# frankyeh/UNet-Studio

Hardware: AMD Instinct MI355X
Metric: voxels/sec 3D U-Net train step @128^3 bf16 (higher is better)
Workload: dtype bf16

## Files before the change

### unet-studio_amd/csrc/device_util.h

```cpp
#pragma once
#include <hip/hip_bf16.h>
#include <hip/hip_runtime.h>
#include <cstdint>

#include "kernels.h"

namespace unet {

typedef __hip_bfloat16 bf16;

template <typename T> __device__ __forceinline__ float ld(const T* p, int64_t i);
template <> __device__ __forceinline__ float ld<float>(const float* p, int64_t i) { return p[i]; }
template <> __device__ __forceinline__ float ld<bf16>(const bf16* p, int64_t i) { return __bfloat162float(p[i]); }
template <typename T> __device__ __forceinline__ void st(T* p, int64_t i, float v);
template <> __device__ __forceinline__ void st<float>(float* p, int64_t i, float v) { p[i] = v; }
template <> __device__ __forceinline__ void st<bf16>(bf16* p, int64_t i, float v) { p[i] = __float2bfloat16(v); }

__device__ __forceinline__ float act_f(float v, int act) {
    switch (act) {
        case 1: return v > 0.f ? v : 0.f;
        case 2: return v > 0.f ? v : 0.01f * v;
        case 3: return v > 0.f ? v : expm1f(v);
        default: return v;
    }
// ... 42 lines not shown
}

constexpr int BRICK_X = 16, BRICK_Y = 4, BRICK_Z = 4;

__device__ __forceinline__ bool brick_walk(int W, int H, int D, int gx, int gy, int& x, int& y, int& z) {
    const unsigned nb = gridDim.x, per = (nb + 7) / 8;
    const unsigned b = (blockIdx.x & 7) * per + (blockIdx.x >> 3);
    if (b >= nb) { x = y = z = 0; return false; }
    const unsigned bx = b % gx, r = b / gx, by = r % gy, bz = r / gy;
    x = bx * BRICK_X + (threadIdx.x & (BRICK_X - 1));
    y = by * BRICK_Y + ((threadIdx.x / BRICK_X) & (BRICK_Y - 1));
    z = bz * BRICK_Z + threadIdx.x / (BRICK_X * BRICK_Y);
    return x < W && y < H && z < D;
}

struct Tri {
    unsigned o[8];
    float tx, ty, tz;
    bool ok;
};

__device__ __forceinline__ Tri locate(float x, float y, float z, int W, int H, int D) {
#pragma clang fp contract(off)
    Tri t;
    t.ok = (x >= 0.f) && (y >= 0.f) && (z >= 0.f) && (x <= (float)(W - 1)) && (y <= (float)(H - 1)) && (z <= (float)(D - 1));
    if (!t.ok) return t;
    float fx = floorf(x), fy = floorf(y), fz = floorf(z);
    t.tx = x - fx; t.ty = y - fy; t.tz = z - fz;
    const int x0 = (int)fx, y0 = (int)fy, z0 = (int)fz;
    const int x1 = min(x0 + 1, W - 1), y1 = min(y0 + 1, H - 1), z1 = min(z0 + 1, D - 1);
    const unsigned r00 = (unsigned)(z0 * H + y0) * (unsigned)W, r10 = (unsigned)(z0 * H + y1) * (unsigned)W,
                   r01 = (unsigned)(z1 * H + y0) * (unsigned)W, r11 = (unsigned)(z1 * H + y1) * (unsigned)W;
    t.o[0] = r00 + x0; t.o[1] = r00 + x1; t.o[2] = r10 + x0; t.o[3] = r10 + x1;
    t.o[4] = r01 + x0; t.o[5] = r01 + x1; t.o[6] = r11 + x0; t.o[7] = r11 + x1;
    return t;
}

__device__ __forceinline__ float lerp1(float t, float a, float b) {
#pragma clang fp contract(off)
    return a + t * (b - a);
}

__device__ __forceinline__ float trilinear(const Tri& t, const float* __restrict__ vol) {
    float c00 = lerp1(t.tx, vol[t.o[0]], vol[t.o[1]]);
    float c10 = lerp1(t.tx, vol[t.o[2]], vol[t.o[3]]);
    float c01 = lerp1(t.tx, vol[t.o[4]], vol[t.o[5]]);
    float c11 = lerp1(t.tx, vol[t.o[6]], vol[t.o[7]]);
    return lerp1(t.tz, lerp1(t.ty, c00, c10), lerp1(t.ty, c01, c11));
}

__device__ __forceinline__ float majority(const Tri& t, const float* __restrict__ vol) {
#pragma clang fp contract(off)
    float v[8], w[8];
    float wx[2] = {1.0f - t.tx, t.tx}, wy[2] = {1.0f - t.ty, t.ty}, wz[2] = {1.0f - t.tz, t.tz};
#pragma unroll
    for (int i = 0; i < 8; ++i) {
        v[i] = vol[t.o[i]];
        w[i] = wx[i & 1] * wy[(i >> 1) & 1] * wz[i >> 2];
    }
    float best = v[0], best_score = -1.f;
#pragma unroll
    for (int j = 0; j < 8; ++j) {
        float s = 0.f;
#pragma unroll
        for (int i = 0; i < 8; ++i) s += (v[i] == v[j]) ? w[i] : 0.f;
        if (s > best_score) { best_score = s; best = v[j]; }
    }
    return best;
}

__device__ __forceinline__ void pp_acc(float x, float& m, float& s, float& sf, float fgc) {
    if (x > m) {
        const float e = expf(m - x);
        s = s * e + 1.f;
        sf = sf * e + fgc;
        m = x;
    } else if (x != -INFINITY) {
        const float e = expf(x - m);
        s += e;
        sf += fgc * e;
    }
}

static inline unsigned cdiv64(int64_t a, int64_t b) { return (unsigned)((a + b - 1) / b); }

}
```

### unet-studio_amd/csrc/engine.cpp

```cpp
#include <hip/hip_runtime.h>

#include <algorithm>
#include <atomic>
#include <cmath>
#include <cstdio>
#include <cstring>
#include <functional>
#include <stdexcept>
#include <string>
#include <mutex>
#include <random>
#include <unordered_map>
#include <vector>

#include "../../include/unet_hip.h"
#include "conv_select.h"
#include "graph.hpp"
#include "kernels.h"

using namespace unet;

namespace {

thread_local std::string g_err;
int fail(const std::string& m) { g_err = m; return 1; }

#define HIP_OK(expr)                                                                              \
    do {                                                                                          \
        hipError_t e_ = (expr);                                                                   \
        if (e_ != hipSuccess) throw std::runtime_error(std::string(#expr) + ": " + hipGetErrorString(e_)); \
    } while (0)

struct DeviceGuard {
    int prev = -1;
    explicit DeviceGuard(int dev) {
        HIP_OK(hipGetDevice(&prev));
        if (prev != dev) HIP_OK(hipSetDevice(dev));
        else prev = -1;
    }
    ~DeviceGuard() { if (prev >= 0) (void)hipSetDevice(prev); }
};

size_t align_up(size_t v, size_t a = 256) { return (v + a - 1) / a * a; }

struct EnvSwitches {
    bool no_side_stream = getenv("UNET_NO_SIDE_STREAM"), no_first_wgrad_fuse = getenv("UNET_NO_FIRST_WGRAD_FUSE"), op_polite = getenv("UNET_OP_POLITE");
};
const EnvSwitches& env() { static const EnvSwitches e; return e; }

struct ProfRec { int op, cat; hipEvent_t e0, e1; };
struct ProfSink { std::vector<ProfRec> recs; };
thread_local ProfSink* g_prof = nullptr;
struct ProfScope {
    ProfRec r{};
    hipStream_t s = nullptr;
    bool on = false;
    ProfScope(int op, int cat, hipStream_t st) {
        if (!g_prof) return;
        on = true; s = st; r.op = op; r.cat = cat;
        if (hipEventCreate(&r.e0) != hipSuccess || hipEventCreate(&r.e1) != hipSuccess) { on = false; return; }
        (void)hipEventRecord(r.e0, s);
    }
    ~ProfScope() {
        if (!on) return;
        (void)hipEventRecord(r.e1, s);
        g_prof->recs.push_back(r);
    }
};

}

struct unet_plan {
    Graph g;
    int dtype = 0, device = 0, impl = 0;
    size_t elsize = 4;
    std::vector<size_t> t_off, g_off;
    std::vector<size_t> a_off;
    std::vector<size_t> n_stat, n_coef;
    std::vector<size_t> w_fwd, w_dgrad;
    std::vector<size_t> wm_fwd, wm_dgrad;
    std::vector<int> n_consumers;
    std::vector<int> first_consumer;
    mutable std::mutex bn_mu;
    mutable std::unordered_map<const void*, std::pair<int, int>> bn_pending;
    mutable std::unordered_map<const void*, std::vector<int>> bn_done;
    std::vector<ConvChoice> conv;
    size_t wgrad_off = 0;
    std::vector<size_t> wz_off;
    std::vector<int> wz_job_of_op;
    std::vector<WgradReduceJob> wz_jobs;
    WgradReduceJob* wz_jobs_dev = nullptr;
    size_t partial_off = 0, partial_bytes = 0;
    size_t ws_bytes = 0;
    size_t loss_bytes = 0;
    std::vector<int64_t> p_off;
    std::vector<PackJob> pack_jobs;
    int64_t pack_blocks = 0;
    PackJob* jobs_dev = nullptr;
    SgdSeg* segs_dev = nullptr;
    int nseg = 0;
    int64_t n_param_elems = 0;

    hipStream_t side = nullptr;
    hipEvent_t ev_fork = nullptr, ev_join = nullptr, ev_pack = nullptr, ev_packd = nullptr;
    int pack_split_op = 0;
    int64_t pack_split_blocks = 0, pack_fwd_blocks = 0;
    size_t head_off = 0;
    size_t deep_part_off = 0, deep_part_bytes = 0, deep_cnt_off = 0;
    static constexpr int deep_ncnt = 4096;
    std::vector<size_t> head_op_off;

    ~unet_plan() {
        if (segs_dev) (void)hipFree(segs_dev);
        if (wz_jobs_dev) (void)hipFree(wz_jobs_dev);
        if (jobs_dev) (void)hipFree(jobs_dev);
        if (ev_fork) (void)hipEventDestroy(ev_fork);
        if (ev_join) (void)hipEventDestroy(ev_join);
        if (ev_pack) (void)hipEventDestroy(ev_pack);
        if (ev_packd) (void)hipEventDestroy(ev_packd);
        if (side) (void)hipStreamDestroy(side);
    }

    ConvGeom op_geom_of(const Op& op) const {
        const Tensor& a = g.tensors[op.src[0]];
        const Tensor& o = g.tensors[op.dst];
        ConvGeom cg;
        cg.Cin = op.cin; cg.Cout = op.cout; cg.D = a.D; cg.H = a.H; cg.W = a.W; cg.Do = o.D; cg.Ho = o.H; cg.Wo = o.W;
        cg.ks = op.ks; cg.stride = op.stride;
        return cg;
    }
    void src_chans(const Op& op, SrcDesc* sd) const {
        for (int k = 0; k < op.nsrc; ++k) sd[k].C = g.tensors[op.src[k]].C;
    }
    std::vector<int> side_polite;
    std::vector<char> wgrad_on_main;
    void choose_polite() {
        side_polite.assign(g.ops.size(), 0);
        wgrad_on_main.assign(g.ops.size(), 0);
        bool first = true, any_deep = false;
        for (size_t i = 0; i < g.ops.size(); ++i) {
            const Op& op = g.ops[i];
            if (op.kind != OP_CONV && op.kind != OP_CONVT) continue;
            if (g.tensors[op.dst].voxels() <= (int64_t)32 * 32 * 32) { any_deep = true; break; }
            if (!first && op.kind == OP_CONV && op.stride == 2) wgrad_on_main[i] = 1;
            first = false;
        }
        if (!any_deep) return;
        for (size_t i = 0; i < g.ops.size(); ++i) {
            const Op& op = g.ops[i];
            if (op.kind == OP_CONV || op.kind == OP_CONVT) side_polite[i] = wgrad_on_main[i] ? 0 : 1;
        }
    }

    bool head_only(size_t t) const {
        if (dtype != UNET_DTYPE_BF16 || g.tensors[t].norm < 0 || g.tensors[t].C % 16) return false;
        int readers = 0;
        for (size_t i = 0; i < g.ops.size(); ++i) {
            const Op& op = g.ops[i];
            if (op.kind == OP_NORM) continue;
            for (int k = 0; k < op.nsrc; ++k) {
                if (op.src[k] != (int)t) continue;
                if (conv[i].fwd != Fwd::head) return false;
                ++readers;
            }
        }
        return readers > 0;
    }
    void layout() {
        choose_polite();
        conv.assign(g.ops.size(), ConvChoice());
        for (size_t i = 0; i < g.ops.size(); ++i) {
            const Op& op = g.ops[i];
            if (op.kind != OP_CONV && op.kind != OP_CONVT) continue;
            SrcDesc sd[2];
            src_chans(op, sd);
            conv[i] = choose_conv(dtype, impl, op_geom_of(op), sd, op.nsrc, op.out_level >= 0, op.kind == OP_CONVT);
        }
        size_t off = 0;
        auto take = [&](size_t bytes) { size_t o = off; off = align_up(off + bytes); return o; };
        t_off.assign(g.tensors.size(), SIZE_MAX);
        g_off.assign(g.tensors.size(), SIZE_MAX);
        n_consumers.assign(g.tensors.size(), 0);
        first_consumer.assign(g.tensors.size(), -1);
        for (size_t oi = 0; oi < g.ops.size(); ++oi) {
            const Op& op = g.ops[oi];
            for (int k = 0; k < op.nsrc && op.kind != OP_NORM; ++k)
                if (op.src[k] >= 0) { ++n_consumers[op.src[k]]; if (first_consumer[op.src[k]] < 0) first_consumer[op.src[k]] = (int)oi; }
        }
        a_off.assign(g.tensors.size(), SIZE_MAX);
        for (size_t i = 0; i < g.tensors.size(); ++i) {
            t_off[i] = take((size_t)g.tensors[i].numel() * elsize);
            if (g.tensors[i].needs_grad) g_off[i] = take((size_t)g.tensors[i].numel() * elsize);
            if (impl == UNET_IMPL_AUTO && (g.tensors[i].norm >= 0 || g.tensors[i].act != ACT_NONE) && !head_only(i))
                a_off[i] = take((size_t)g.tensors[i].numel() * elsize);
        }
        n_stat.resize(g.norms.size()); n_coef.resize(g.norms.size());
        size_t pmax = 0;
        for (size_t i = 0; i < g.norms.size(); ++i) {
            n_stat[i] = take(4 * (size_t)g.norms[i].C * 4);
            n_coef[i] = take(3 * (size_t)g.norms[i].C * 4);
            size_t pb = (size_t)stats_blocks(g.tensors[g.norms[i].tensor].voxels()) * g.norms[i].C * 2 * (dtype == UNET_DTYPE_F32 ? 8 : 4);
            if (pb > pmax) pmax = pb;
        }
        w_fwd.assign(g.ops.size(), SIZE_MAX); w_dgrad.assign(g.ops.size(), SIZE_MAX);
        wm_fwd.assign(g.ops.size(), SIZE_MAX); wm_dgrad.assign(g.ops.size(), SIZE_MAX);
        auto grow = [](size_t& m, size_t b) { if (b > m) m = b; };
        for (size_t i = 0; i < g.ops.size(); ++i) {
            const Op& op = g.ops[i];
            if (op.kind != OP_CONV && op.kind != OP_CONVT) continue;
            const ConvChoice& c = conv[i];
            const ConvGeom cg = op_geom_of(op);
            int k3 = op.kind == OP_CONV ? op.ks * op.ks * op.ks : 8;
            w_fwd[i] = take((size_t)k3 * op.cin * round_up(op.cout, 8) * 4);
            w_dgrad[i] = take((size_t)k3 * op.cout * round_up(op.cin, 8) * 4);
            if (op.kind == OP_CONVT) {
                if (c.mfma_fwd()) { wm_fwd[i] = take(mfma_convt_w_bytes(cg)); wm_dgrad[i] = take(mfma_convt_dgrad_w_bytes(cg)); }
                continue;
            }
            const bool stats = g.tensors[op.dst].norm >= 0;
            SrcDesc sd[2];
            src_chans(op, sd);
            if (c.mfma_fwd()) {
                wm_fwd[i] = take(mfma_conv_w_bytes(cg));
                if (stats) grow(pmax, (size_t)mfma_conv_blocks(cg) * op.cout * 2 * 4);
            }
            if (c.fwd == Fwd::first_f32_mfma && stats) grow(pmax, (size_t)conv_first_f32_mfma_blocks(cg) * op.cout * 2 * 8);
            if (c.fwd == Fwd::f32_mfma && stats) grow(pmax, (size_t)conv_f32_mfma_stat_rows(cg, sd) * op.cout * 2 * 8);
            if (c.dgrad == Dgrad::mfma) {
                wm_dgrad[i] = take(mfma_conv_dgrad_w_bytes(cg));
                if (op.stride == 2) grow(pmax, (size_t)s2_conv_dgrad_rows_max() * op.cin * 2 * 4);
            }
        }
        partial_bytes = pmax ? pmax : 256;
        partial_off = take(partial_bytes);
        size_t wmax = 0, hmax = 0;
        for (size_t i = 0; i < g.ops.size(); ++i) {
            const Op& op = g.ops[i];
            if (op.kind != OP_CONV && op.kind != OP_CONVT) continue;
            const ConvChoice& c = conv[i];
            const ConvGeom cg = op_geom_of(op);
            grow(wmax, wgrad_direct_scratch_bytes(cg, op.kind == OP_CONVT));
            if (op.kind == OP_CONVT) {
                if (c.wgrad == Wgrad::mfma) {
                    grow(wmax, mfma_convt_wgrad_scratch_bytes(cg));
                    grow(wmax, bias_grad_scratch_bytes(cg.Cout, (int64_t)cg.Do * cg.Ho * cg.Wo));
                }
                continue;
            }
            if (c.wgrad == Wgrad::mfma) grow(wmax, mfma_wgrad_scratch_bytes(cg, side_polite[i]));
            if (c.wgrad == Wgrad::f32_mfma) grow(wmax, wgrad_f32_mfma_scratch_bytes(cg));
            if (wgrad_small_supported(cg, op.nsrc)) grow(wmax, wgrad_small_scratch_bytes(cg));
            if (cg.Cin == 1 && (cg.Cout == 16 || cg.Cout == 32)) grow(wmax, conv_first_wgrad_mfma_scratch_bytes(cg));
            if (head_supported(cg, op.nsrc)) grow(hmax, head_bwd_scratch_bytes(cg));
        }
        wgrad_off = take(wmax ? wmax : 256);
        head_off = take(hmax ? hmax : 256);
        if (dtype == UNET_DTYPE_BF16 && impl == UNET_IMPL_AUTO) {
            deep_part_bytes = (size_t)8 << 20;
            deep_part_off = take(deep_part_bytes);
            deep_cnt_off = take((size_t)deep_ncnt * 4);
        }
        head_op_off.assign(g.ops.size(), SIZE_MAX);
        for (size_t i = 0; i < g.ops.size(); ++i)
            if (conv[i].fwd == Fwd::head) head_op_off[i] = take(head_bwd_scratch_bytes(op_geom_of(g.ops[i])));
        wz_off.assign(g.ops.size(), SIZE_MAX);
        for (size_t i = 0; i < g.ops.size(); ++i) {
            const Op& op = g.ops[i];
            const Wgrad w = conv[i].wgrad;
            if (op.out_level >= 0 || (w != Wgrad::first_mfma && w != Wgrad::mfma)) continue;
            const ConvGeom cg = op_geom_of(op);
            if (w == Wgrad::first_mfma) wz_off[i] = take(conv_first_wgrad_mfma_scratch_bytes(cg));
            else if (op.kind == OP_CONV) { if (!mfma_conv_wgrad_direct(cg)) wz_off[i] = take(mfma_wgrad_scratch_bytes(cg, side_polite[i])); }
            else if (!mfma_convt_wgrad_direct(cg)) wz_off[i] = take(mfma_convt_wgrad_scratch_bytes(cg));
        }
        ws_bytes = off;
        p_off.assign(g.params.size() + 1, 0);
        for (size_t i = 0; i < g.params.size(); ++i) {
            int64_t n = 1;
            for (auto d : g.params[i].shape) n *= d;
            p_off[i + 1] = p_off[i] + n;
        }
        wz_jobs.clear();
        wz_job_of_op.assign(g.ops.size(), -1);
        int wz_blk = 0;
        for (size_t i = 0; i < g.ops.size(); ++i) {
            if (wz_off[i] == SIZE_MAX) continue;
            const Op& op = g.ops[i];
            ConvGeom cg = op_geom_of(op);
            WgradReduceJob j;
            j.op = (int)i;
            j.slab_off = (long long)(wz_off[i] / 4);
            j.dw_off = p_off[op.weight];
            j.Cb = op.cout;
            if (op.kind == OP_CONVT) {
                j.nsplit = mfma_convt_wgrad_splits(cg);
                j.n = (long long)8 * op.cin * op.cout;
                j.bias_off = op.bias >= 0 ? j.slab_off + (long long)j.nsplit * j.n : -1;
                j.db_off = op.bias >= 0 ? p_off[op.bias] : -1;
            } else {
                j.nsplit = conv[i].wgrad == Wgrad::first_mfma ? conv_first_wgrad_splits(cg) : mfma_conv_wgrad_splits(cg, side_polite[i]);
                j.n = (long long)27 * op.cin * op.cout;
                j.bias_off = op.bias >= 0 ? j.slab_off + (long long)j.nsplit * j.n : -1;
                j.db_off = op.bias >= 0 ? p_off[op.bias] : -1;
            }
            wz_blk += wgrad_reduce_job_blocks(j, wz_blk);
            wz_job_of_op[i] = (int)wz_jobs.size();
            wz_jobs.push_back(j);
        }
        pack_jobs.clear();
        pack_blocks = 0;
        pack_split_op = -1; pack_split_blocks = 0; pack_fwd_blocks = 0;
        for (int which = 0; which < 2; ++which) {
            for (size_t i = 0; i < g.ops.size(); ++i) {
                const Op& op = g.ops[i];
                if (!conv[i].mfma_fwd()) continue;
                if (which == 0 && pack_split_op < 0 && g.tensors[op.dst].voxels() <= (int64_t)16 * 16 * 16) { pack_split_op = (int)i; pack_split_blocks = pack_blocks; }
                PackJob jb[2];
                int n = op.kind == OP_CONV ? mfma_conv_pack_jobs(op_geom_of(op), conv[i].dgrad == Dgrad::mfma, jb) : mfma_convt_pack_jobs(op_geom_of(op), jb);
                if (which >= n) continue;
                jb[which].src_off = p_off[op.weight];
                jb[which].dst_off = (int64_t)(which == 0 ? wm_fwd[i] : wm_dgrad[i]);
                jb[which].blk0 = pack_blocks;
                pack_blocks += jb[which].total;
                pack_jobs.push_back(jb[which]);
            }
            if (which == 0) pack_fwd_blocks = pack_blocks;
        }
    }
};

namespace {

void norm_fwd_passes(int dtype, const void* raw, int C, int64_t S, float* partial, int rows, bool dbl, bool eval, const float* gamma,
                     const float* beta, double eps, float* stat, float* rm, float* rv, int act, void* act_out, hipStream_t s) {
    if (eval) launch_norm_eval(C, gamma, beta, rm, rv, eps, stat, s);
    else {
        if (!rows) {
            launch_stats_partial(dtype, raw, C, S, partial, s);
            rows = stats_blocks(S);
            dbl = dtype == UNET_DTYPE_F32;
        }
        if (!dbl && act_out && launch_norm_finalize_apply(dtype, partial, rows, C, S, gamma, beta, eps, stat, rm, rv, 0.1, raw, act, act_out, s))
            return;
        launch_norm_finalize(partial, rows, C, S, gamma, beta, eps, stat, rm, rv, 0.1, s, dbl);
    }
    if (act_out) {
        SrcDesc d;
        d.ptr = raw; d.C = C; d.act = act; d.scale = stat + 2 * C; d.shift = stat + 3 * C;
        launch_apply_view(dtype, d, act_out, S, s);
    }
}
void norm_bwd_passes(int dtype, void* g, const void* u, int C, int64_t S, const float* stat, int act, const float* gamma, float* coef,
                     float* dgamma, float* dbeta, float* partial, int rows, bool no_apply, hipStream_t s) {
    if (rows <= 0) {
        launch_norm_bwd_partial(dtype, g, u, C, S, stat, act, partial, s);
        rows = stats_blocks(S);
    }
    if (!no_apply && launch_norm_bwd_finalize_apply(dtype, partial, rows, C, S, gamma, stat, coef, dgamma, dbeta, g, u, act, s)) return;
    launch_norm_bwd_finalize(partial, rows, C, S, gamma, stat, coef, dgamma, dbeta, s, dtype == UNET_DTYPE_F32);
    if (!no_apply) launch_norm_bwd_apply(dtype, g, u, C, S, stat, coef, act, s);
}

struct Exec {
    const unet_plan& p;
    char* ws;
    hipStream_t s;
    bool deep_on = false;
    Exec(const unet_plan& plan, void* workspace, void* stream) : p(plan), ws((char*)workspace), s((hipStream_t)stream) {}
    DeepScratch deep() const {
        DeepScratch d;
        if (deep_on && p.deep_part_bytes) { d.part = (float*)(ws + p.deep_part_off); d.part_bytes = p.deep_part_bytes; d.cnt = (int*)(ws + p.deep_cnt_off); d.ncnt = p.deep_ncnt; }
        return d;
    }
    int* deep_cnt() const { return p.deep_part_bytes ? (int*)(ws + p.deep_cnt_off) : nullptr; }

    void* tptr(int t) const { return ws + p.t_off[t]; }
    void* gptr(int t) const { return p.g_off[t] == SIZE_MAX ? nullptr : ws + p.g_off[t]; }
    float* stat(int n) const { return (float*)(ws + p.n_stat[n]); }
    float* coef(int n) const { return (float*)(ws + p.n_coef[n]); }
    float* partial() const { return (float*)(ws + p.partial_off); }

    SrcDesc raw_src(int t) const {
        const Tensor& T = p.g.tensors[t];
        SrcDesc d;
        d.ptr = tptr(t); d.C = T.C; d.act = T.act;
        if (T.norm >= 0) { d.scale = stat(T.norm) + 2 * T.C; d.shift = stat(T.norm) + 3 * T.C; }
        return d;
    }
    SrcDesc src(int t) const {
        if (p.a_off[t] == SIZE_MAX) return raw_src(t);
        SrcDesc d;
        d.ptr = ws + p.a_off[t]; d.C = p.g.tensors[t].C;
        return d;
    }
    void apply_view(int t) const {
        if (p.a_off[t] != SIZE_MAX) launch_apply_view(p.dtype, raw_src(t), ws + p.a_off[t], p.g.tensors[t].voxels(), s);
    }
    ConvGeom geom(const Op& op) const { return p.op_geom_of(op); }

    void forward(const float* const* params, float* const* buffers, const float* x, float* const* outs, int mode,
                 const std::function<void(int)>* on_head = nullptr) {
        const Graph& g = p.g;
        const bool packs_current = (mode & UNET_MODE_PACKS_CURRENT) != 0;
        mode &= 1;
        std::vector<int> fused_blocks(g.norms.size(), 0);
        std::vector<char> fused_dbl(g.norms.size(), 0);
        std::vector<char> fused_done(g.norms.size(), 0);
        bool packed = false, pack_pending = false, pack2_pending = false;
        if (p.jobs_dev && packs_current) { packed = true; deep_on = true; }
        else if (p.jobs_dev) {
            bool flat = true;
            for (size_t i = 0; i < g.params.size() && flat; ++i) flat = params[i] == params[0] + p.p_off[i];
            if (flat) {
                const int njobs = (int)p.pack_jobs.size();
                if (mode == 1 && p.side && !env().no_side_stream && !g_prof) {
                    HIP_OK(hipEventRecord(p.ev_fork, s));
                    HIP_OK(hipStreamWaitEvent(p.side, p.ev_fork, 0));
                    if (p.pack_split_op > 0 && p.pack_split_blocks > 0) {
                        launch_mfma_pack_batched(params[0], ws, p.jobs_dev, njobs, p.pack_split_blocks, p.side, 0, 0, deep_cnt(), p.deep_ncnt);
                        HIP_OK(hipEventRecord(p.ev_join, p.side));
                        launch_mfma_pack_batched(params[0], ws, p.jobs_dev, njobs, p.pack_fwd_blocks - p.pack_split_blocks, p.side, p.pack_split_blocks);
                        HIP_OK(hipEventRecord(p.ev_pack, p.side));
                        pack2_pending = true;
                        launch_mfma_pack_batched(params[0], ws, p.jobs_dev, njobs, p.pack_blocks - p.pack_fwd_blocks, p.side, p.pack_fwd_blocks);
                        HIP_OK(hipEventRecord(p.ev_packd, p.side));
                    } else {
                        launch_mfma_pack_batched(params[0], ws, p.jobs_dev, njobs, p.pack_blocks, p.side, 0, 0, deep_cnt(), p.deep_ncnt);
                        HIP_OK(hipEventRecord(p.ev_join, p.side));
                    }
                    pack_pending = true;
                } else {
                    ProfScope ps(-1, UNET_PROF_OTHER, s);
                    launch_mfma_pack_batched(params[0], ws, p.jobs_dev, njobs, mode == 1 ? p.pack_blocks : p.pack_fwd_blocks, s, 0, 0, deep_cnt(), p.deep_ncnt);
                }
                packed = true;
                deep_on = true;
            }
        }
        auto need_packs = [&](int op_index = 1 << 30) {
            if (pack_pending) { HIP_OK(hipStreamWaitEvent(s, p.ev_join, 0)); pack_pending = false; }
            if (pack2_pending && op_index >= p.pack_split_op) { HIP_OK(hipStreamWaitEvent(s, p.ev_pack, 0)); pack2_pending = false; }
        };
        for (size_t i = 0; i < g.ops.size(); ++i) {
            const Op& op = g.ops[i];
            ProfScope ps((int)i, (op.kind == OP_CONV || op.kind == OP_CONVT) ? UNET_PROF_CONV_FWD : op.kind == OP_NORM ? UNET_PROF_NORM_FWD : UNET_PROF_OTHER, s);
            switch (op.kind) {
                case OP_PACK_INPUT:
                    launch_pack_input(p.dtype, x, tptr(op.dst), g.in_c, g.tensors[op.dst].voxels(), s);
                    break;
                case OP_CONV:
                case OP_CONVT: {
                    if (op.out_level >= 0 && !(outs && outs[op.out_level])) break;
                    SrcDesc sd[2] = {src(op.src[0]), op.nsrc > 1 ? src(op.src[1]) : SrcDesc()};
                    ConvGeom cg = geom(op);
                    float* wf = (float*)(ws + p.w_fwd[i]);
                    float* wd = (float*)(ws + p.w_dgrad[i]);
                    const int k3 = op.ks * op.ks * op.ks;
                    const ConvChoice& c = p.conv[i];
                    const Tensor& T = g.tensors[op.dst];
                    const bool want_stats = T.norm >= 0 && !(g.norms[T.norm].batch && mode == 0);
                    if (op.kind == OP_CONVT) {
                        if (c.mfma_fwd()) {
                            need_packs((int)i);
                            if (!packed) launch_mfma_pack_convt_w(params[op.weight], ws + p.wm_fwd[i], mode == 1 ? ws + p.wm_dgrad[i] : nullptr, cg, s);
                            if (!(deep_on && launch_deep_convt_fwd(cg, sd, op.nsrc, ws + p.wm_fwd[i], params[op.bias], tptr(op.dst), deep(), s)))
                                launch_mfma_convt_fwd(cg, sd, op.nsrc, ws + p.wm_fwd[i], params[op.bias], tptr(op.dst), s);
                            break;
                        }
                        if (!packs_current) launch_pack_convt_w(params[op.weight], wf, wd, op.cin, op.cout, s);
                        if (c.fwd == Fwd::f32_mfma) launch_convt_f32_mfma(cg, sd, wf, params[op.bias], (float*)tptr(op.dst), s);
                        else launch_convt_fwd_direct(p.dtype, cg, sd, op.nsrc, wf, params[op.bias], tptr(op.dst), s);
                        break;
                    }
                    float* const part = want_stats ? partial() : nullptr;
                    int rows = 0;
                    switch (c.fwd) {
                        case Fwd::deep:
                        case Fwd::mfma:
                            need_packs((int)i);
                            if (!packed)
                                launch_mfma_pack_conv_w(params[op.weight], ws + p.wm_fwd[i],
                                                        (mode == 1 && c.dgrad == Dgrad::mfma) ? ws + p.wm_dgrad[i] : nullptr, cg, s);
                            if (mode == 1 && c.dgrad != Dgrad::mfma && !packs_current) launch_pack_conv_w(params[op.weight], wf, wd, op.cin, op.cout, k3, s);
                            if (c.fwd == Fwd::deep && deep_on) {
                                DeepNormFwd nf;
                                const bool fuse = T.norm >= 0 && p.a_off[op.dst] != SIZE_MAX;
                                if (fuse) {
                                    const Norm& n = g.norms[T.norm];
                                    nf = {params[n.gamma], params[n.beta], n.eps, stat(T.norm), n.batch ? buffers[n.buffer] : nullptr,
                                          n.batch ? buffers[n.buffer + 1] : nullptr, 0.1, (n.batch && mode == 0) ? 1 : 0, T.act, ws + p.a_off[op.dst]};
                                }
                                if (launch_deep_conv_fwd(cg, sd, op.nsrc, ws + p.wm_fwd[i], params[op.bias], tptr(op.dst), fuse ? &nf : nullptr, deep(), s)) {
                                    if (fuse) fused_done[T.norm] = 1;
                                    break;
                                }
                            }
                            rows = launch_mfma_conv_fwd(cg, sd, op.nsrc, ws + p.wm_fwd[i], params[op.bias], tptr(op.dst), part, s);
                            break;
                        case Fwd::head:
                            launch_head_fwd(p.dtype, cg, sd[0], params[op.weight], params[op.bias], outs[op.out_level] ? nullptr : tptr(op.dst),
                                            outs[op.out_level], s);
                            break;
                        case Fwd::first_mfma:
                            rows = launch_conv_first_mfma(cg, sd, params[op.weight], params[op.bias], tptr(op.dst), part, s);
                            if (mode == 1 && !packs_current && g.tensors[op.src[0]].needs_grad)
                                launch_pack_conv_w(params[op.weight], wf, wd, op.cin, op.cout, k3, s);
                            break;
                        case Fwd::first_f32_mfma:
                            rows = launch_conv_first_f32_mfma(cg, sd, params[op.weight], params[op.bias], (float*)tptr(op.dst), (double*)part, s);
                            if (mode == 1 && !packs_current) launch_pack_conv_w(params[op.weight], wf, wd, op.cin, op.cout, k3, s);
                            break;
                        case Fwd::f32_mfma:
                            if (!packs_current) launch_pack_conv_w(params[op.weight], wf, wd, op.cin, op.cout, k3, s);
                            rows = launch_conv_f32_mfma(cg, sd, op.nsrc, wf, params[op.bias], (float*)tptr(op.dst), s, (double*)part);
                            break;
                        case Fwd::direct:
                            if (!packs_current) launch_pack_conv_w(params[op.weight], wf, wd, op.cin, op.cout, k3, s);
                            launch_conv_fwd_direct(p.dtype, cg, sd, op.nsrc, wf, params[op.bias], tptr(op.dst),
                                                   op.out_level >= 0 ? outs[op.out_level] : nullptr, s);
                            break;
                    }
                    if (want_stats) {
                        fused_blocks[T.norm] = rows;
                        fused_dbl[T.norm] = c.fwd == Fwd::first_f32_mfma || c.fwd == Fwd::f32_mfma;
                    }
                    break;
                }
                case OP_NORM: {
                    const Norm& n = g.norms[op.norm];
                    const Tensor& T = g.tensors[n.tensor];
                    if (fused_done[op.norm]) break;
                    norm_fwd_passes(p.dtype, tptr(n.tensor), n.C, T.voxels(), partial(), fused_blocks[op.norm], fused_dbl[op.norm] != 0,
                                    n.batch && mode == 0, params[n.gamma], params[n.beta], n.eps, stat(op.norm),
                                    n.batch ? buffers[n.buffer] : nullptr, n.batch ? buffers[n.buffer + 1] : nullptr, T.act,
                                    p.a_off[n.tensor] != SIZE_MAX ? ws + p.a_off[n.tensor] : nullptr, s);
                    break;
                }
                case OP_MATERIALIZE: {
                    SrcDesc sd[2] = {src(op.src[0]), op.nsrc > 1 ? src(op.src[1]) : SrcDesc()};
                    launch_materialize(p.dtype, sd, op.nsrc, tptr(op.dst), g.tensors[op.dst].voxels(), s);
                    break;
                }
                case OP_MAXPOOL: {
                    const Tensor& a = g.tensors[op.src[0]];
                    launch_maxpool_fwd(p.dtype, src(op.src[0]), tptr(op.dst), a.D, a.H, a.W, s);
                    break;
                }
                case OP_UPSAMPLE: {
                    const Tensor& a = g.tensors[op.src[0]];
                    launch_upsample_fwd(p.dtype, src(op.src[0]), tptr(op.dst), a.D, a.H, a.W, s);
                    break;
                }
                case OP_EXPORT:
                    if (outs && outs[op.out_level])
                        launch_export(p.dtype, src(op.src[0]), outs[op.out_level], g.tensors[op.src[0]].voxels(), s);
                    break;
            }
            if (op.kind != OP_NORM && op.kind != OP_EXPORT && op.dst >= 0) {
                const Tensor& T = g.tensors[op.dst];
                if (T.norm < 0 && T.act != ACT_NONE) apply_view(op.dst);
            }
            if (on_head && op.out_level >= 0 && outs && outs[op.out_level] && (op.kind == OP_CONV || op.kind == OP_CONVT || op.kind == OP_EXPORT))
                (*on_head)(op.out_level);
        }
        need_packs();
    }

    void view_backward(int t, const float* const* params, float* const* gparams, bool no_apply = false) {
        const Tensor& T = p.g.tensors[t];
        if (T.norm >= 0) {
            const Norm& n = p.g.norms[T.norm];
            int have = 0;
            {
                std::lock_guard<std::mutex> lk(p.bn_mu);
                auto d = p.bn_done.find(ws);
                if (d != p.bn_done.end()) {
                    auto f = std::find(d->second.begin(), d->second.end(), t);
                    if (f != d->second.end()) { d->second.erase(f); return; }
                }
                auto it = p.bn_pending.find(ws);
                if (it != p.bn_pending.end()) { if (it->second.first == t) have = it->second.second; p.bn_pending.erase(it); }
            }
            norm_bwd_passes(p.dtype, gptr(t), tptr(t), T.C, T.voxels(), stat(T.norm), T.act, params[n.gamma], coef(T.norm),
                            gparams[n.gamma], gparams[n.beta], partial(), have, no_apply, s);
        } else if (T.act != ACT_NONE) {
            launch_act_bwd(p.dtype, gptr(t), tptr(t), T.act, T.numel(), s);
        }
    }

    void backward(const float* const* params, const float* const* grad_outs, float* const* gparams, float* grad_x, int op_hi = 1 << 30,
                  int op_lo = 0) {
        const Graph& g = p.g;
        if (p.side) HIP_OK(hipStreamWaitEvent(s, p.ev_packd, 0));
        {
            bool flat = p.jobs_dev != nullptr;
            for (size_t k = 0; k < g.params.size() && flat; ++k) flat = params[k] == params[0] + p.p_off[k];
            deep_on = flat;
        }
        std::vector<char> init(g.tensors.size(), 0);
        auto dst_of = [&](int t) {
            DstGrad d;
            d.C = g.tensors[t].C;
            d.ptr = g.tensors[t].needs_grad ? gptr(t) : nullptr;
            d.accumulate = init[t];
            return d;
        };
        auto mark = [&](const Op& op) {
            for (int k = 0; k < op.nsrc; ++k)
                if (g.tensors[op.src[k]].needs_grad) init[op.src[k]] = 1;
        };
        const hipStream_t sb = (p.side && !env().no_side_stream && !g_prof) ? p.side : s;
        auto fork = [&]() {
            if (sb == s) return;
            HIP_OK(hipEventRecord(p.ev_fork, s));
            HIP_OK(hipStreamWaitEvent(sb, p.ev_fork, 0));
        };
        if (op_lo < 0) op_lo = 0;
        if (op_hi >= (int)g.ops.size()) { std::lock_guard<std::mutex> lk(p.bn_mu); p.bn_pending.erase(ws); p.bn_done.erase(ws); }
// ... 720 lines not shown
        g.stride = 2; g.Do = (D - 1) / 2 + 1; g.Ho = (H - 1) / 2 + 1; g.Wo = (W - 1) / 2 + 1;
        w = std::max(mfma_wgrad_scratch_bytes(g, 0), mfma_wgrad_scratch_bytes(g, 1));
        if (w > b) b = w;
        g.Do = 2 * D; g.Ho = 2 * H; g.Wo = 2 * W;
        w = mfma_convt_wgrad_scratch_bytes(g);
        if (w > b) b = w;
    }
    *bytes = b;
    return 0;
}

static ConvGeom op_geom(int cin, int cout, int D, int H, int W, int ks, int stride, bool transposed) {
    ConvGeom g;
    g.Cin = cin; g.Cout = cout; g.D = D; g.H = H; g.W = W; g.ks = ks; g.stride = stride;
    if (transposed) { g.Do = 2 * D; g.Ho = 2 * H; g.Wo = 2 * W; }
    else {
        int pad = (ks - 1) / 2;
        g.Do = (D + 2 * pad - ks) / stride + 1; g.Ho = (H + 2 * pad - ks) / stride + 1; g.Wo = (W + 2 * pad - ks) / stride + 1;
    }
    return g;
}
static void op_pack(const float* w, int cin, int cout, int k3, bool transposed, void* scratch, float** wf, float** wd, hipStream_t s) {
    *wf = (float*)scratch; *wd = (float*)((char*)scratch + OpScratch(cin, cout).half);
    if (transposed) launch_pack_convt_w(w, *wf, *wd, cin, cout, s);
    else launch_pack_conv_w(w, *wf, *wd, cin, cout, k3, s);
}
#define OP_TRY(...) try { __VA_ARGS__; check_launch(); return 0; } catch (const std::exception& e) { return fail(e.what()); }
static DeepScratch op_deep() {
    static std::mutex mu;
    static std::unordered_map<int, DeepScratch> per_dev;
    int dev = 0;
    HIP_OK(hipGetDevice(&dev));
    std::lock_guard<std::mutex> lk(mu);
    auto it = per_dev.find(dev);
    if (it != per_dev.end()) return it->second;
    DeepScratch d;
    d.part_bytes = (size_t)8 << 20; d.ncnt = 4096;
    char* base = nullptr;
    HIP_OK(hipMalloc((void**)&base, d.part_bytes + (size_t)d.ncnt * 4));
    HIP_OK(hipMemset(base + d.part_bytes, 0, (size_t)d.ncnt * 4));
    d.part = (float*)base; d.cnt = (int*)(base + d.part_bytes);
    per_dev[dev] = d;
    return d;
}

int unet_op_conv3d_fwd(int dtype, int impl, const void* x, const float* w, const float* b, void* y, int cin, int cout, int D, int H,
                       int W, int ks, int stride, void* scratch, void* stream) {
    OP_TRY({
        hipStream_t s = (hipStream_t)stream;
        ConvGeom g = op_geom(cin, cout, D, H, W, ks, stride, false);
        float *wf, *wd;
        SrcDesc sd; sd.ptr = x; sd.C = cin;
        const ConvChoice c = choose_conv(dtype, impl, g, &sd, 1, false, false);
        if (c.mfma_fwd()) {
            void* wm = (char*)scratch + OpScratch(cin, cout).pack;
            launch_mfma_pack_conv_w(w, wm, nullptr, g, s);
            if (!launch_deep_conv_fwd(g, &sd, 1, wm, b, y, nullptr, op_deep(), s)) launch_mfma_conv_fwd(g, &sd, 1, wm, b, y, nullptr, s);
        } else if (c.fwd == Fwd::first_mfma) {
            launch_conv_first_mfma(g, &sd, w, b, y, nullptr, s);
        } else if (c.fwd == Fwd::first_f32_mfma) {
            (void)launch_conv_first_f32_mfma(g, &sd, w, b, (float*)y, nullptr, s);
        } else {
            op_pack(w, cin, cout, ks * ks * ks, false, scratch, &wf, &wd, s);
            if (c.fwd == Fwd::f32_mfma) (void)launch_conv_f32_mfma(g, &sd, 1, wf, b, (float*)y, s);
            else launch_conv_fwd_direct(dtype, g, &sd, 1, wf, b, y, nullptr, s);
        }
    })
}
int unet_op_conv3d_fwd_fused(int dtype, int impl, const void* x, const float* scale, const float* shift, int act, const float* w,
                             const float* b, void* y, float* stats, int cin, int cout, int D, int H, int W, int ks, int stride,
                             void* scratch, void* stream) {
    OP_TRY({
        hipStream_t s = (hipStream_t)stream;
        ConvGeom g = op_geom(cin, cout, D, H, W, ks, stride, false);
        float *wf, *wd;
        SrcDesc sd; sd.ptr = x; sd.C = cin; sd.scale = scale; sd.shift = shift; sd.act = act;
        int64_t So = (int64_t)g.Do * g.Ho * g.Wo;
        const OpScratch L(cin, cout);
        float* part = (float*)((char*)scratch + L.partials);
        const ConvChoice c = choose_conv(dtype, impl, g, &sd, 1, false, false);
        if (c.mfma_fwd()) {
            void* wm = (char*)scratch + L.pack;
            launch_mfma_pack_conv_w(w, wm, nullptr, g, s);
            int rows = launch_mfma_conv_fwd(g, &sd, 1, wm, b, y, stats ? part : nullptr, s);
            if (stats) launch_stats_sum(part, rows, cout, stats, s);
        } else if (c.fwd == Fwd::first_mfma) {
            int rows = launch_conv_first_mfma(g, &sd, w, b, y, stats ? part : nullptr, s);
            if (stats) launch_stats_sum(part, rows, cout, stats, s);
        } else {
            op_pack(w, cin, cout, ks * ks * ks, false, scratch, &wf, &wd, s);
            if (c.fwd == Fwd::f32_mfma) {
                const int rows = launch_conv_f32_mfma(g, &sd, 1, wf, b, (float*)y, s, stats ? (double*)part : nullptr);
                if (stats) launch_stats_sum(part, rows, cout, stats, s, true);
            } else {
                launch_conv_fwd_direct(dtype, g, &sd, 1, wf, b, y, nullptr, s);
                if (stats) {
                    launch_stats_partial(dtype, y, cout, So, part, s);
                    launch_stats_sum(part, stats_blocks(So), cout, stats, s, dtype == UNET_DTYPE_F32);
                }
            }
        }
    })
}
int unet_op_conv3d_pack(int dtype, const float* w, void* wpacked, int cin, int cout, int D, int H, int W, int ks, int stride,
                        void* stream) {
    OP_TRY({
        ConvGeom g = op_geom(cin, cout, D, H, W, ks, stride, false);
        SrcDesc sd; sd.C = cin;
        if (!choose_conv(dtype, UNET_IMPL_AUTO, g, &sd, 1, false, false).mfma_fwd())
            throw std::runtime_error("unet_op_conv3d_pack: shape not covered by the MFMA kernels");
        launch_mfma_pack_conv_w(w, wpacked, nullptr, g, (hipStream_t)stream);
    })
}
int unet_op_conv3d_fwd_packed(int dtype, const void* x, const void* wpacked, const float* b, void* y, float* stats_partials,
                              int cin, int cout, int D, int H, int W, int ks, int stride, void* stream) {
    OP_TRY({
        ConvGeom g = op_geom(cin, cout, D, H, W, ks, stride, false);
        SrcDesc sd; sd.ptr = x; sd.C = cin;
        if (!choose_conv(dtype, UNET_IMPL_AUTO, g, &sd, 1, false, false).mfma_fwd())
            throw std::runtime_error("unet_op_conv3d_fwd_packed: shape not covered by the MFMA kernels");
        launch_mfma_conv_fwd(g, &sd, 1, wpacked, b, y, stats_partials, (hipStream_t)stream);
    })
}
int unet_op_conv3d_bwd_data(int dtype, int impl, const void* dy, const float* w, void* dx, int cin, int cout, int D, int H, int W,
                            int ks, int stride, void* scratch, void* stream) {
    OP_TRY({
        hipStream_t s = (hipStream_t)stream;
        ConvGeom g = op_geom(cin, cout, D, H, W, ks, stride, false);
        float *wf, *wd;
        DstGrad d; d.ptr = dx; d.C = cin; d.accumulate = 0;
        SrcDesc sd; sd.C = cin;
        const Dgrad c = choose_conv(dtype, impl, g, &sd, 1, false, false).dgrad;
        if (c == Dgrad::mfma) {
            void* wm = (char*)scratch + OpScratch(cin, cout).pack;
            launch_mfma_pack_conv_w(w, nullptr, wm, g, s);
            if (!launch_deep_conv_dgrad(g, dy, wm, &d, 1, nullptr, op_deep(), s)) launch_mfma_conv_dgrad(g, dy, wm, &d, 1, s);
        } else {
            op_pack(w, cin, cout, ks * ks * ks, false, scratch, &wf, &wd, s);
            if (c == Dgrad::f32_mfma) launch_conv_f32_mfma_dgrad(g, (const float*)dy, wd, &d, 1, s);
            else launch_conv_dgrad_direct(dtype, g, dy, wd, &d, 1, s);
        }
    })
}
int unet_op_conv3d_fwd_norm(const void* x0, const void* x1, int cin0, int cin1, const float* w, const float* b, const float* gamma,
                            const float* beta, double eps, float* rm, float* rv, double momentum, int use_running, int act, void* y,
                            void* y_act, float* stat, int cout, int D, int H, int W, int stride, void* scratch, void* stream) {
    OP_TRY({
        hipStream_t s = (hipStream_t)stream;
        const int cin = cin0 + cin1, nsrc = x1 ? 2 : 1;
        ConvGeom g = op_geom(cin, cout, D, H, W, 3, stride, false);
        SrcDesc sd[2];
        sd[0].ptr = x0; sd[0].C = cin0;
        if (x1) { sd[1].ptr = x1; sd[1].C = cin1; }
        const ConvChoice c = choose_conv(UNET_DTYPE_BF16, UNET_IMPL_AUTO, g, sd, nsrc, false, false);
        if (!c.mfma_fwd() || (use_running && (!rm || !rv)))
            throw std::runtime_error("unet_op_conv3d_fwd_norm: shape not covered by the MFMA kernels, or eval mode without running statistics");
        const OpScratch L(cin, cout);
        void* wm = (char*)scratch + L.pack;
        float* part = (float*)((char*)scratch + L.partials);
        launch_mfma_pack_conv_w(w, wm, nullptr, g, s);
        const DeepNormFwd nf = {gamma, beta, eps, stat, rm, rv, momentum, use_running ? 1 : 0, act, y_act};
        if (!(c.fwd == Fwd::deep && launch_deep_conv_fwd(g, sd, nsrc, wm, b, y, &nf, op_deep(), s))) {
            const int rows = launch_mfma_conv_fwd(g, sd, nsrc, wm, b, y, use_running ? nullptr : part, s);
            norm_fwd_passes(UNET_DTYPE_BF16, y, cout, (int64_t)g.Do * g.Ho * g.Wo, part, rows, false, use_running != 0, gamma, beta, eps,
                            stat, rm, rv, act, y_act, s);
        }
    })
}
int unet_op_conv3d_bwd_data_norm(int transposed, const void* dy, const float* w, void* dx, int accumulate, const void* u, const float* stat,
                                 const float* gamma, int act, float* coef, float* dgamma, float* dbeta, int cin, int cout, int D, int H,
                                 int W, void* scratch, void* stream) {
    OP_TRY({
        hipStream_t s = (hipStream_t)stream;
        ConvGeom g = op_geom(cin, cout, D, H, W, transposed ? 2 : 3, transposed ? 2 : 1, transposed != 0);
        SrcDesc sd; sd.C = cin;
        if (choose_conv(UNET_DTYPE_BF16, UNET_IMPL_AUTO, g, &sd, 1, false, transposed != 0).dgrad != Dgrad::mfma)
            throw std::runtime_error("unet_op_conv3d_bwd_data_norm: shape not covered by the MFMA kernels");
        const OpScratch L(cin, cout);
        void* wm = (char*)scratch + L.pack;
        float* part = (float*)((char*)scratch + L.partials);
        DstGrad d; d.ptr = dx; d.C = cin; d.accumulate = accumulate ? 1 : 0;
        const DeepNormBwd nb = {u, stat, gamma, coef, dgamma, dbeta, act};
        bool done = false;
        int rows = 0;
        if (transposed) {
            launch_mfma_pack_convt_w(w, nullptr, wm, g, s);
            int norm_done = 0;
            if (launch_deep_convt_dgrad(g, dy, wm, &d, 1, &nb, op_deep(), &norm_done, s)) done = norm_done != 0;
            else launch_mfma_convt_dgrad(g, dy, wm, &d, 1, s);
        } else {
            launch_mfma_pack_conv_w(w, nullptr, wm, g, s);
            const BnBwdStats bn = {u, stat, part, act, cin};
            const int served = launch_deep_conv_dgrad(g, dy, wm, &d, 1, &nb, op_deep(), s);
            done = served == 2;
            if (!served) rows = launch_mfma_conv_dgrad(g, dy, wm, &d, 1, s, &bn);
        }
        if (!done) norm_bwd_passes(UNET_DTYPE_BF16, dx, u, cin, (int64_t)D * H * W, stat, act, gamma, coef, dgamma, dbeta, part, rows, false, s);
    })
}
int unet_op_conv3d_bwd_weight(int dtype, int impl, const void* x, const void* dy, float* dw, float* db, int cin, int cout, int D,
                              int H, int W, int ks, int stride, void* scratch, void* stream) {
    OP_TRY({
        hipStream_t s = (hipStream_t)stream;
        ConvGeom g = op_geom(cin, cout, D, H, W, ks, stride, false);
        SrcDesc sd; sd.ptr = x; sd.C = cin;
        switch (choose_conv(dtype, impl, g, &sd, 1, false, false).wgrad) {
            case Wgrad::first_mfma: launch_conv_first_wgrad_mfma(g, &sd, dy, dw, db, scratch, s); break;
            case Wgrad::mfma: launch_mfma_conv_wgrad(g, &sd, 1, dy, dw, db, scratch, s, false, env().op_polite ? 1 : 0); break;
            case Wgrad::f32_mfma: launch_wgrad_f32_mfma(g, &sd, 1, (const float*)dy, dw, db, scratch, s); break;
            case Wgrad::small: launch_conv_wgrad_small(dtype, g, &sd, 1, dy, dw, db, scratch, s); break;
            case Wgrad::direct: launch_conv_wgrad_direct(dtype, g, &sd, 1, dy, dw, db, nullptr, s);
        }
    })
}
int unet_op_convt_fwd(int dtype, int impl, const void* x, const float* w, const float* b, void* y, int cin, int cout, int D, int H,
                      int W, void* scratch, void* stream) {
    OP_TRY({
        hipStream_t s = (hipStream_t)stream;
        ConvGeom g = op_geom(cin, cout, D, H, W, 2, 2, true);
        float *wf, *wd;
        SrcDesc sd; sd.ptr = x; sd.C = cin;
        const Fwd f = choose_conv(dtype, impl, g, &sd, 1, false, true).fwd;
        if (f == Fwd::mfma) {
            void* wm = (char*)scratch + OpScratch(cin, cout).pack;
            launch_mfma_pack_convt_w(w, wm, nullptr, g, s);
            if (!launch_deep_convt_fwd(g, &sd, 1, wm, b, y, op_deep(), s)) launch_mfma_convt_fwd(g, &sd, 1, wm, b, y, s);
        } else {
            op_pack(w, cin, cout, 8, true, scratch, &wf, &wd, s);
            if (f == Fwd::f32_mfma) launch_convt_f32_mfma(g, &sd, wf, b, (float*)y, s);
            else launch_convt_fwd_direct(dtype, g, &sd, 1, wf, b, y, s);
        }
    })
}
int unet_op_convt_bwd_data(int dtype, int impl, const void* dy, const float* w, void* dx, int cin, int cout, int D, int H, int W,
                           void* scratch, void* stream) {
    OP_TRY({
        hipStream_t s = (hipStream_t)stream;
        ConvGeom g = op_geom(cin, cout, D, H, W, 2, 2, true);
        float *wf, *wd;
        DstGrad d; d.ptr = dx; d.C = cin; d.accumulate = 0;
        SrcDesc sd; sd.C = cin;
        if (choose_conv(dtype, impl, g, &sd, 1, false, true).dgrad == Dgrad::mfma) {
            void* wm = (char*)scratch + OpScratch(cin, cout).pack;
            launch_mfma_pack_convt_w(w, nullptr, wm, g, s);
            if (!launch_deep_convt_dgrad(g, dy, wm, &d, 1, nullptr, op_deep(), nullptr, s)) launch_mfma_convt_dgrad(g, dy, wm, &d, 1, s);
        } else {
            op_pack(w, cin, cout, 8, true, scratch, &wf, &wd, s);
            launch_convt_dgrad_direct(dtype, g, dy, wd, &d, 1, s);
// ... 458 lines not shown
```

### unet-studio_amd/csrc/kernels.h

```cpp
#pragma once
#include <hip/hip_runtime.h>
#include <cstdint>

#include "../../include/unet_atlas.h"
#include "../../include/unet_augment.h"
#include "../../include/unet_components.h"
#include "../../include/unet_feed.h"
#include "../../include/unet_hip.h"
#include "../../include/unet_postproc.h"
#include "../../include/unet_preproc.h"
#include "../../include/unet_qc.h"
#include "../../include/unet_space.h"
#include "../../include/unet_tiles.h"

namespace unet {

struct SrcDesc {
    const void* ptr = nullptr;
    int C = 0;
    const float* scale = nullptr;
    const float* shift = nullptr;
    int act = 0;
};
struct DstGrad {
    void* ptr = nullptr;
    int C = 0;
    int accumulate = 0;
};

struct ConvGeom {
    int Cin = 0, Cout = 0;
    int D = 0, H = 0, W = 0;
    int Do = 0, Ho = 0, Wo = 0;
    int ks = 3, stride = 1;
};

__host__ __device__ static inline int round_up(int a, int b) { return (a + b - 1) / b * b; }

void launch_pack_conv_w(const float* w, float* w_fwd, float* w_dgrad, int Cin, int Cout, int k3, hipStream_t s);
void launch_pack_convt_w(const float* w, float* w_fwd, float* w_dgrad, int Cin, int Cout, hipStream_t s);

void launch_pack_input(int dtype, const float* x_ncdhw, void* y, int C, int64_t S, hipStream_t s);
void launch_export(int dtype, SrcDesc src, float* y_ncdhw, int64_t S, hipStream_t s);
void launch_import_grad(int dtype, const float* g_ncdhw, void* g, int C, int64_t S, int accumulate, hipStream_t s);

void launch_conv_fwd_direct(int dtype, const ConvGeom& g, const SrcDesc* src, int nsrc, const float* w_fwd, const float* bias,
                            void* out, float* out_ncdhw, hipStream_t s);
void launch_conv_dgrad_direct(int dtype, const ConvGeom& g, const void* dy, const float* w_dgrad, const DstGrad* dst, int ndst,
                              hipStream_t s);
size_t wgrad_direct_scratch_bytes(const ConvGeom& g, int transposed);
void launch_conv_wgrad_direct(int dtype, const ConvGeom& g, const SrcDesc* src, int nsrc, const void* dy, float* dw, float* db,
                              void* scratch, hipStream_t s);
void launch_convt_fwd_direct(int dtype, const ConvGeom& g, const SrcDesc* src, int nsrc, const float* w_fwd, const float* bias,
                             void* out, hipStream_t s);
void launch_convt_dgrad_direct(int dtype, const ConvGeom& g, const void* dy, const float* w_dgrad, const DstGrad* dst, int ndst,
                               hipStream_t s);
void launch_convt_wgrad_direct(int dtype, const ConvGeom& g, const SrcDesc* src, int nsrc, const void* dy, float* dw, float* db,
                               void* scratch, hipStream_t s);

int stats_blocks(int64_t S);
void launch_stats_partial(int dtype, const void* x, int C, int64_t S, float* partial, hipStream_t s);
void launch_norm_finalize(const float* partial, int nblk, int C, int64_t S, const float* gamma, const float* beta, double eps,
                          float* stat, float* running_mean, float* running_var, double momentum, hipStream_t s, bool dbl = false);
void launch_stats_sum(const float* partial, int nblk, int C, float* out, hipStream_t s, bool dbl = false);
void launch_norm_eval(int C, const float* gamma, const float* beta, const float* rm, const float* rv, double eps, float* stat,
                      hipStream_t s);

void launch_act_bwd(int dtype, void* g, const void* u, int act, int64_t n, hipStream_t s);
void launch_norm_bwd_partial(int dtype, void* g, const void* u, int C, int64_t S, const float* stat, int act, float* partial,
                             hipStream_t s);
void launch_norm_bwd_finalize(const float* partial, int nblk, int C, int64_t S, const float* gamma, const float* stat, float* coef,
                              float* dgamma, float* dbeta, hipStream_t s, bool dbl = false);
bool launch_norm_finalize_apply(int dtype, const float* partial, int nblk, int C, int64_t S, const float* gamma, const float* beta, double eps,
                                float* stat, float* running_mean, float* running_var, double momentum, const void* raw, int act, void* out,
                                hipStream_t s);
bool launch_norm_bwd_finalize_apply(int dtype, const float* partial, int nblk, int C, int64_t S, const float* gamma, const float* stat,
                                    float* coef, float* dgamma, float* dbeta, void* g, const void* u, int act, hipStream_t s);
void launch_norm_bwd_apply(int dtype, void* g, const void* u, int C, int64_t S, const float* stat, const float* coef, int act,
                           hipStream_t s);

void launch_maxpool_fwd(int dtype, SrcDesc src, void* out, int D, int H, int W, hipStream_t s);
void launch_maxpool_bwd(int dtype, SrcDesc src, const void* gout, DstGrad dst, int D, int H, int W, hipStream_t s);
void launch_upsample_fwd(int dtype, SrcDesc src, void* out, int D, int H, int W, hipStream_t s);
void launch_upsample_bwd(int dtype, const void* gout, DstGrad dst, int D, int H, int W, hipStream_t s);
void launch_materialize(int dtype, const SrcDesc* src, int nsrc, void* out, int64_t S, hipStream_t s);
void launch_apply_view(int dtype, SrcDesc src, void* out, int64_t S, hipStream_t s);
void launch_materialize_bwd(int dtype, const void* gout, const DstGrad* dst, int ndst, int64_t S, hipStream_t s);
void launch_export_bwd(int dtype, const float* g_ncdhw, DstGrad dst, int64_t S, hipStream_t s);
void launch_unpack_ncdhw(int dtype, const void* g, float* out_ncdhw, int C, int64_t S, hipStream_t s);

void launch_target_half(const int64_t* t, int64_t* o, int D, int H, int W, hipStream_t s);
int loss_blocks(int64_t S);
void launch_loss_partial(const float* logits, const int64_t* target, int C, int64_t S, int collapse, float* partial, hipStream_t s);
void launch_loss_finalize(const float* partial, int nblk, int oc, float level_weight, int cost_mask, float* level_out, float* totals,
                          int set_stats, hipStream_t s);
void launch_loss_grad(const float* logits, const int64_t* target, int C, int64_t S, int collapse, const float* level_out,
                      float level_weight, int cost_mask, float* dlogits, hipStream_t s);

void launch_sum_buffers(const float* const* bufs, int n, float* out, int64_t count, int zero_inputs, hipStream_t s);

struct SgdSeg { int64_t offset, count; float wd; };
void launch_sumsq_partial(const float* g, int64_t n, float scale, float* partial, int nblk, hipStream_t s);
void launch_sgd(float* p, float* g, float* m, int64_t n, const SgdSeg* segs_dev, int nseg, const float* partial, int nblk,
                float lr, float momentum, int nesterov, float weight_decay, float clip_norm, float grad_scale, float* norm_out,
                hipStream_t s);

struct PackJob { int64_t src_off, dst_off, total, blk0; int Ci, Co, CK, T, mode, A, B, pad; };
int mfma_conv_pack_jobs(const ConvGeom& g, bool want_dgrad, PackJob* out2);
int mfma_convt_pack_jobs(const ConvGeom& g, PackJob* out2);
void launch_mfma_pack_batched(const float* params_base, void* ws, const PackJob* jobs_dev, int njobs, int64_t nblocks, hipStream_t s,
                              int64_t blk_base = 0, int max_grid = 0, int* zero = nullptr, int nzero = 0);
bool mfma_conv_fwd_supported(int dtype, const ConvGeom& g, const SrcDesc* src, int nsrc);
size_t mfma_conv_w_bytes(const ConvGeom& g);
void launch_mfma_pack_conv_w(const float* w, void* w_mfma_fwd, void* w_mfma_dgrad, const ConvGeom& g, hipStream_t s);
int launch_mfma_conv_fwd(const ConvGeom& g, const SrcDesc* src, int nsrc, const void* w_mfma, const float* bias, void* out,
                         float* stats_partial, hipStream_t s);
bool conv_first_mfma_supported(int dtype, const ConvGeom& g, const SrcDesc* src, int nsrc);
int conv_first_mfma_blocks(const ConvGeom& g);
int launch_conv_first_mfma(const ConvGeom& g, const SrcDesc* src, const float* w, const float* bias, void* out, float* stats_partial,
                           hipStream_t s);
int mfma_conv_blocks(const ConvGeom& g);
bool mfma_wgrad_z_supported(int dtype, const ConvGeom& g, const SrcDesc* src, int nsrc);
size_t mfma_wgrad_z_scratch_bytes(const ConvGeom& g, int polite = 0);
int mfma_wgrad_z_splits(const ConvGeom& g, int polite = 0);
int launch_mfma_wgrad_z(const ConvGeom& g, const SrcDesc* src, int nsrc, const void* dy, bool want_bias, void* scratch, hipStream_t s,
                        int polite = 0);
void wgrad_reduce(const float* slab, const float* bias_slab, int nsplit, int64_t n, int Cb, float* dw, float* db, hipStream_t s);
struct WgradReduceJob { long long slab_off, bias_off, dw_off, db_off, n; int nsplit, Cb, ly, blk0, nblk, op; };
int wgrad_reduce_job_blocks(WgradReduceJob& j, int blk0);
void launch_wgrad_reduce_batched(const WgradReduceJob* jobs_dev, int job0, int njobs, int blk_base, int nblocks, const void* ws, float* gflat,
                                 hipStream_t s);
bool mfma_wgrad_supported(int dtype, const ConvGeom& g, const SrcDesc* src, int nsrc);
size_t mfma_wgrad_scratch_bytes(const ConvGeom& g, int polite = 0);
int mfma_conv_wgrad_splits(const ConvGeom& g, int polite = 0);
int mfma_convt_wgrad_splits(const ConvGeom& g);
bool mfma_conv_wgrad_direct(const ConvGeom& g);
bool mfma_convt_wgrad_direct(const ConvGeom& g);
int conv_first_wgrad_splits(const ConvGeom& g);
void launch_mfma_conv_wgrad(const ConvGeom& g, const SrcDesc* src, int nsrc, const void* dy, float* dw, float* db, void* scratch,
                            hipStream_t s, bool defer_reduce = false, int polite = 0);
bool head_supported(const ConvGeom& g, int nsrc);
size_t head_bwd_scratch_bytes(const ConvGeom& g);
void launch_head_fwd(int dtype, const ConvGeom& g, const SrcDesc& src, const float* w, const float* bias, void* y, float* out_ncdhw,
                     hipStream_t s);
void launch_head_bwd(int dtype, const ConvGeom& g, const SrcDesc& src, const float* dy_ncdhw, const void* dy_cl, const float* w,
                     DstGrad dst, float* dw, float* db, void* scratch, hipStream_t s, bool defer_reduce = false);
void launch_head_bwd_reduce(const ConvGeom& g, float* dw, float* db, const void* scratch, hipStream_t s);
// ... 130 lines not shown
```

### unet-studio_amd/csrc/kernels_elem.hip

```cpp
#include "device_util.h"

namespace unet {

template <typename T> __global__ void k_pack_input(const float* __restrict__ x, T* __restrict__ y, int C, int64_t S) {
    int64_t i = (int64_t)blockIdx.x * 256 + threadIdx.x;
    if (i >= S * C) return;
    int c = (int)(i % C); int64_t v = i / C;
    st<T>(y, i, x[(int64_t)c * S + v]);
}
void launch_pack_input(int dtype, const float* x, void* y, int C, int64_t S, hipStream_t s) {
    UNET_DISPATCH(dtype, (k_pack_input<T><<<cdiv64(S * C, 256), 256, 0, s>>>(x, (T*)y, C, S)));
}

template <typename T> __global__ void k_export(SrcDesc src, float* __restrict__ y, int64_t S) {
    int64_t i = (int64_t)blockIdx.x * 256 + threadIdx.x;
    if (i >= S * src.C) return;
    int c = (int)(i / S); int64_t v = i % S;
    y[i] = view_ld<T>(src, v, c);
}
void launch_export(int dtype, SrcDesc src, float* y, int64_t S, hipStream_t s) {
    UNET_DISPATCH(dtype, (k_export<T><<<cdiv64(S * src.C, 256), 256, 0, s>>>(src, y, S)));
}
void launch_unpack_ncdhw(int dtype, const void* g, float* out, int C, int64_t S, hipStream_t s) {
    SrcDesc d;
    d.ptr = g; d.C = C;
    launch_export(dtype, d, out, S, s);
}

template <typename T> __global__ void k_import_grad(const float* __restrict__ g, T* __restrict__ o, int C, int64_t S, int acc) {
    int64_t i = (int64_t)blockIdx.x * 256 + threadIdx.x;
    if (i >= S * C) return;
    int c = (int)(i % C); int64_t v = i / C;
    float val = g[(int64_t)c * S + v];
    if (acc) val += ld<T>(o, i);
    st<T>(o, i, val);
}
void launch_import_grad(int dtype, const float* g, void* o, int C, int64_t S, int accumulate, hipStream_t s) {
    UNET_DISPATCH(dtype, (k_import_grad<T><<<cdiv64(S * C, 256), 256, 0, s>>>(g, (T*)o, C, S, accumulate)));
}
void launch_export_bwd(int dtype, const float* g, DstGrad dst, int64_t S, hipStream_t s) {
    if (!dst.ptr) return;
    launch_import_grad(dtype, g, dst.ptr, dst.C, S, dst.accumulate, s);
}

static inline int64_t stats_vpb(int64_t S) {
    int64_t vpb = (S + 1023) / 1024;
    return vpb < 32 ? 32 : vpb;
}
int stats_blocks(int64_t S) {
    int64_t vpb = stats_vpb(S);
    return (int)((S + vpb - 1) / vpb);
}
static inline int pow2_ge(int c) { int p = 1; while (p < c && p < 256) p <<= 1; return p; }

template <typename T> struct StatAcc { typedef float type; };
template <> struct StatAcc<float> { typedef double type; };

template <typename T, int MODE>
__global__ void __launch_bounds__(256) k_stats_partial(const T* __restrict__ x, T* __restrict__ gbuf, int C, int64_t S, int64_t VPB,
                                                       int CW, const float* __restrict__ stat, int act, float* __restrict__ partial_) {
    typedef typename StatAcc<T>::type A;
    A* partial = (A*)partial_;
    __shared__ A red[2][256];
    int NV = 256 / CW, cl = threadIdx.x % CW, lane = threadIdx.x / CW;
    int64_t v0 = (int64_t)blockIdx.x * VPB, v1 = v0 + VPB < S ? v0 + VPB : S;
    for (int cg = 0; cg < C; cg += CW) {
        int c = cg + cl;
        A s1 = 0, s2 = 0;
        if (c < C) {
            float mean = 0.f, rstd = 1.f, sc = 1.f, sh = 0.f;
            if (MODE == 1) { mean = stat[c]; rstd = stat[C + c]; sc = stat[2 * C + c]; sh = stat[3 * C + c]; }
            for (int64_t v = v0 + lane; v < v1; v += NV) {
                float u = ld<T>(x, v * C + c);
                if (MODE == 0) { s1 += (A)u; s2 += (A)u * (A)u; }
                else {
                    float dv = ld<T>(gbuf, v * C + c) * act_d(fmaf(u, sc, sh), act);
                    s1 += (A)dv; s2 += (A)dv * (A)((u - mean) * rstd);
                }
            }
        }
        red[0][threadIdx.x] = s1; red[1][threadIdx.x] = s2;
        __syncthreads();
        if (lane == 0 && c < C) {
            A a = 0, b = 0;
            for (int l = 0; l < NV; ++l) { a += red[0][l * CW + cl]; b += red[1][l * CW + cl]; }
            partial[((int64_t)blockIdx.x * C + c) * 2 + 0] = a;
            partial[((int64_t)blockIdx.x * C + c) * 2 + 1] = b;
        }
        __syncthreads();
    }
}
void launch_stats_partial(int dtype, const void* x, int C, int64_t S, float* partial, hipStream_t s) {
    int nb = stats_blocks(S);
    UNET_DISPATCH(dtype, (k_stats_partial<T, 0><<<nb, 256, 0, s>>>((const T*)x, nullptr, C, S, stats_vpb(S), pow2_ge(C), nullptr, 0, partial)));
// ... 499 lines not shown
    const int CP = C / 2, RG = CP >= 256 ? 1 : 256 / CP;
    for (int idx = threadIdx.x; idx < CP * RG; idx += 256) {
        const int cp = idx % CP, rg = idx / CP;
        double a0 = 0.0, b0 = 0.0, a1 = 0.0, b1 = 0.0;
        for (int r0 = rg; r0 < nblk; r0 += 16 * RG) {
            float4 v[16];
#pragma unroll
            for (int k = 0; k < 16; ++k) {
                const int r = r0 + k * RG;
                v[k] = r < nblk ? *(const float4*)(partial + ((int64_t)r * C + 2 * cp) * 2) : make_float4(0.f, 0.f, 0.f, 0.f);
            }
#pragma unroll
            for (int k = 0; k < 16; ++k) { a0 += v[k].x; b0 += v[k].y; a1 += v[k].z; b1 += v[k].w; }
        }
        sa[rg * C + 2 * cp] = a0; sb[rg * C + 2 * cp] = b0; sa[rg * C + 2 * cp + 1] = a1; sb[rg * C + 2 * cp + 1] = b1;
    }
    __syncthreads();
    if (RG > 1) {
        for (int c = threadIdx.x; c < C; c += 256) {
            double a = 0.0, b = 0.0;
            for (int q = 0; q < RG; ++q) { a += sa[q * C + c]; b += sb[q * C + c]; }
            sa[c] = a; sb[c] = b;
        }
        __syncthreads();
    }
}
__global__ void __launch_bounds__(256) k_norm_finalize_apply8(const float* __restrict__ partial, int nblk, int C, int64_t S, int64_t VPB,
                                                              const float* __restrict__ gamma, const float* __restrict__ beta, double eps,
                                                              float* __restrict__ stat, float* rm, float* rv, double momentum,
                                                              const uint4* __restrict__ in, int act, uint4* __restrict__ out) {
    __shared__ double sa[FUSED_MAX_C], sb[FUSED_MAX_C];
    __shared__ float s_sc[FUSED_MAX_C], s_sh[FUSED_MAX_C];
    prologue_sums(partial, nblk, C, sa, sb);
    for (int c = threadIdx.x; c < C; c += 256) {
        const double mean = sa[c] / (double)S;
        double var = sb[c] / (double)S - mean * mean;
        if (var < 0.0) var = 0.0;
        const double rstd = 1.0 / sqrt(var + eps), sc = (double)gamma[c] * rstd;
        s_sc[c] = (float)sc; s_sh[c] = (float)((double)beta[c] - mean * sc);
        if (blockIdx.x == 0) {
            stat[c] = (float)mean; stat[C + c] = (float)rstd; stat[2 * C + c] = s_sc[c]; stat[3 * C + c] = s_sh[c];
            if (rm) {
                rm[c] = (float)((1.0 - momentum) * rm[c] + momentum * mean);
                rv[c] = (float)((1.0 - momentum) * rv[c] + momentum * (S > 1 ? var * (double)S / (double)(S - 1) : var));
            }
        }
    }
    __syncthreads();
    const int G8 = C / 8, NV = 256 / G8, grp = threadIdx.x % G8, lane = threadIdx.x / G8, c0 = grp * 8;
    const int64_t v0 = (int64_t)blockIdx.x * VPB, v1 = v0 + VPB < S ? v0 + VPB : S;
    float sc[8], sh[8];
#pragma unroll
    for (int e = 0; e < 8; ++e) { sc[e] = s_sc[c0 + e]; sh[e] = s_sh[c0 + e]; }
    for (int64_t v = v0 + lane; v < v1; v += NV) {
        const uint4 r = in[v * G8 + grp];
        unsigned w[4] = {r.x, r.y, r.z, r.w};
#pragma unroll
        for (int e = 0; e < 4; ++e) {
            float lo = act_f(fmaf(__uint_as_float(w[e] << 16), sc[2 * e], sh[2 * e]), act);
            float hi = act_f(fmaf(__uint_as_float(w[e] & 0xffff0000u), sc[2 * e + 1], sh[2 * e + 1]), act);
            w[e] = (unsigned)__bfloat16_as_ushort(__float2bfloat16(lo)) | ((unsigned)__bfloat16_as_ushort(__float2bfloat16(hi)) << 16);
        }
        out[v * G8 + grp] = make_uint4(w[0], w[1], w[2], w[3]);
    }
}
static inline bool fused_norm_ok(int dtype, int C, int nblk) {
    return dtype == 1 && C % 8 == 0 && C <= FUSED_MAX_C && 256 % (C / 8) == 0 && nblk <= FUSED_MAX_ROWS;
}
static inline int64_t fused_vpb(int C, int64_t S) {
    const int64_t nv = 256 / (C / 8);
    int64_t vpb = (S + 255) / 256;
    if (vpb < 2 * nv) vpb = 2 * nv;
    return (vpb + nv - 1) / nv * nv;
}
bool launch_norm_finalize_apply(int dtype, const float* partial, int nblk, int C, int64_t S, const float* gamma, const float* beta, double eps,
                                float* stat, float* rm, float* rv, double momentum, const void* raw, int act, void* out, hipStream_t s) {
    if (!fused_norm_ok(dtype, C, nblk)) return false;
    const int64_t vpb = fused_vpb(C, S);
    k_norm_finalize_apply8<<<cdiv64(S, vpb), 256, 0, s>>>(partial, nblk, C, S, vpb, gamma, beta, eps, stat, rm, rv, momentum,
                                                          (const uint4*)raw, act, (uint4*)out);
    return true;
}

void launch_materialize(int dtype, const SrcDesc* src, int nsrc, void* out, int64_t S, hipStream_t s) {
    Src2 a;
    a.n = nsrc; a.s[0] = src[0]; if (nsrc > 1) a.s[1] = src[1];
    int C = src[0].C + (nsrc > 1 ? src[1].C : 0);
    UNET_DISPATCH(dtype, (k_materialize<T><<<cdiv64(S * C, 256), 256, 0, s>>>(a, (T*)out, C, S * C)));
}
template <typename T> __global__ void k_materialize_bwd(const T* __restrict__ gout, Dst2 dst, int C, int64_t n) {
    int64_t i = (int64_t)blockIdx.x * 256 + threadIdx.x;
    if (i >= n) return;
    int c = (int)(i % C); int64_t v = i / C;
    int which = (dst.n > 1 && c >= dst.d[0].C) ? 1 : 0;
    const DstGrad& d = dst.d[which];
    if (!d.ptr) return;
    int64_t j = v * d.C + (which ? c - dst.d[0].C : c);
    float val = ld<T>(gout, i);
    T* p = (T*)d.ptr;
    if (d.accumulate) val += ld<T>(p, j);
    st<T>(p, j, val);
}
void launch_materialize_bwd(int dtype, const void* gout, const DstGrad* dst, int ndst, int64_t S, hipStream_t s) {
    Dst2 a;
    a.n = ndst; a.d[0] = dst[0]; if (ndst > 1) a.d[1] = dst[1];
    int C = dst[0].C + (ndst > 1 ? dst[1].C : 0);
    UNET_DISPATCH(dtype, (k_materialize_bwd<T><<<cdiv64(S * C, 256), 256, 0, s>>>((const T*)gout, a, C, S * C)));
}

__global__ void k_target_half(const int64_t* __restrict__ t, int64_t* __restrict__ o, int D, int H, int W) {
    int Do = D >> 1, Ho = H >> 1, Wo = W >> 1;
    int64_t i = (int64_t)blockIdx.x * 256 + threadIdx.x;
    if (i >= (int64_t)Do * Ho * Wo) return;
    int x = (int)(i % Wo); int64_t r = i / Wo;
    int y = (int)(r % Ho); int z = (int)(r / Ho);
    float sd = (float)D / Do, sh = (float)H / Ho, sw = (float)W / Wo;
    int iz = min((int)floorf(z * sd), D - 1), iy = min((int)floorf(y * sh), H - 1), ix = min((int)floorf(x * sw), W - 1);
    o[i] = (int64_t)(float)t[((int64_t)iz * H + iy) * W + ix];
}
void launch_target_half(const int64_t* t, int64_t* o, int D, int H, int W, hipStream_t s) {
    int64_t n = (int64_t)(D >> 1) * (H >> 1) * (W >> 1);
    k_target_half<<<cdiv64(n, 256), 256, 0, s>>>(t, o, D, H, W);
}

int loss_blocks(int64_t S) {
    int64_t nb = (S + 255) / 256;
    return (int)(nb > 1024 ? 1024 : nb);
}

struct VoxelLogits {
    const float* p; int64_t S, v; int k; float lse0;
    __device__ float get(int cp) const { return (k && cp == 0) ? lse0 : p[(int64_t)(k ? cp + k - 1 : cp) * S + v]; }
};
__device__ __forceinline__ VoxelLogits make_vl(const float* logits, int64_t S, int64_t v, int k) {
    VoxelLogits L;
    L.p = logits; L.S = S; L.v = v; L.k = k; L.lse0 = 0.f;
    if (k) {
        float mx = -INFINITY;
        for (int c = 0; c < k; ++c) mx = fmaxf(mx, logits[(int64_t)c * S + v]);
        float s = 0.f;
        for (int c = 0; c < k; ++c) s += __expf(logits[(int64_t)c * S + v] - mx);
        L.lse0 = mx + __logf(s);
    }
    return L;
}
__device__ __forceinline__ float clamp_p(float q) { return fminf(fmaxf(q, 1e-6f), 1.0f - 1e-6f); }

__global__ void __launch_bounds__(256) k_loss_partial(const float* __restrict__ logits, const int64_t* __restrict__ target, int C,
                                                      int64_t S, int k, float* __restrict__ partial) {
    extern __shared__ float sh[];
    int oc = k ? C - k + 1 : C;
    int np = 3 + 2 * oc;
    for (int i = threadIdx.x; i < np; i += 256) sh[i] = 0.f;
    __syncthreads();
    float ce = 0.f, mse = 0.f, nv = 0.f;
    for (int64_t v = (int64_t)blockIdx.x * 256 + threadIdx.x; v < S; v += (int64_t)gridDim.x * 256) {
        int64_t t = target[v];
        bool valid = t < C;
        if (!valid) continue;
        int tt = k ? (int)(t - k + 1 > 0 ? t - k + 1 : 0) : (int)t;
        VoxelLogits L = make_vl(logits, S, v, k);
        float mx = -INFINITY;
        for (int c = 0; c < oc; ++c) mx = fmaxf(mx, L.get(c));
        float sum = 0.f;
        for (int c = 0; c < oc; ++c) sum += __expf(L.get(c) - mx);
        float inv = 1.f / sum, psq = 0.f, pt = 0.f;
// ... 429 lines not shown
```

### unet-studio_amd/csrc/kernels_mfma_conv.hip

```cpp
#include <type_traits>
#include <cstdlib>
#include "mfma_util.h"

namespace unet {

enum PackMode {
    PK_CONV_FWD = 0,
    PK_CONV_DGRAD = 1,
    PK_CONVT_DGRAD = 2,
    PK_CONVT_FWD = 3,
    PK_CONV_S2_DGRAD = 4
};
constexpr int PACK_LDS_ELEMS = 16 * (32 * 27 + 1);
template <int CK, int T, int MODE>
__device__ __forceinline__ void pack_unit_t(const float* __restrict__ w, __bf16* __restrict__ out, int unit, int Co, int A, int B, __bf16* lds) {
    constexpr int KSTEPS = CK == 32 ? T : (T + 1) / 2;
    const int NTT = Co / 16;
    const int q = unit / NTT, nt = unit % NTT, o0 = nt * 16;
    constexpr int RS = CK * T + 1;
    constexpr int n = 16 * CK * T, U = 8;
    for (int e0 = threadIdx.x; e0 < n; e0 += 256 * U) {
        float v[U];
        int dst[U];
#pragma unroll
// ... 333 lines not shown
                for (int n = 0; n < NT; ++n) {
                    int c = (nt0 + n) * 16 + gq * 4;
                    c -= c / a.sc_C * a.sc_C;
                    float b4[4] = {0.f, 0.f, 0.f, 0.f};
                    if (a.bias) {
#pragma unroll
                        for (int r = 0; r < 4; ++r) b4[r] = a.bias[c + r];
                    }
#pragma unroll
                    for (int i = 0; i < MTW; ++i) {
                        if (pp[i][n]) {
                            uint2 o;
                            o.x = pack_bf16x2(acc[i][n][0] + b4[0] + bf_lo(old[i][n].x), acc[i][n][1] + b4[1] + bf_hi(old[i][n].x));
                            o.y = pack_bf16x2(acc[i][n][2] + b4[2] + bf_lo(old[i][n].y), acc[i][n][3] + b4[3] + bf_hi(old[i][n].y));
                            *pp[i][n] = o;
                        }
                        acc[i][n] = f32x4{0.f, 0.f, 0.f, 0.f};
                    }
                }
                continue;
            }
        }
#pragma unroll
        for (int n = 0; n < NT; ++n) {
            int c = (nt0 + n) * 16 + gq * 4;
            int tz = 0, ty = 0, tx = 0;
            if (SC) { int tap = c / a.sc_C; c -= tap * a.sc_C; tz = tap >> 2; ty = (tap >> 1) & 1; tx = tap & 1; }
            float b4[4] = {0.f, 0.f, 0.f, 0.f};
            if (a.bias) {
#pragma unroll
                for (int r = 0; r < 4; ++r) b4[r] = a.bias[c + r];
            }
            int d = (a.nout > 1 && c >= a.outC[0]) ? 1 : 0;
            int cd = c - (d ? a.outC[0] : 0);
            char* obase = (char*)(d ? a.out[1] : a.out[0]);
            const int oC = d ? a.outC[1] : a.outC[0], oacc = d ? a.out_acc[1] : a.out_acc[0];
            const bool edge = z0 + BZ > a.oD || y0 + BY > a.oH || x0 + BX > a.oW;
            char* tbase = obase + ((((long long)z0 * a.oH + y0) * a.oW + x0) * oC + cd) * 2;
#pragma unroll
            for (int i = 0; i < MTW; ++i) {
                const int mt = wave * MTW + i;
                int gz = z0 + mt / (BY / TYM), gy = y0 + (mt % (BY / TYM)) * TYM + (j / TXM), gx = x0 + j % TXM;
                if (SC) { gz = 2 * gz + tz; gy = 2 * gy + ty; gx = 2 * gx + tx; }
                if (((!SC && !edge) || (gz < a.oD && gy < a.oH && gx < a.oW)) && obase) {
                    uint2* p;
                    if (SC) p = (uint2*)(obase + ((((size_t)gz * a.oH + gy) * a.oW + gx) * oC + cd) * 2);
                    else p = (uint2*)(tbase + __umul24(mvox[i], (unsigned)oC * 2));
                    float v0 = acc[i][n][0] + b4[0], v1 = acc[i][n][1] + b4[1], v2 = acc[i][n][2] + b4[2], v3 = acc[i][n][3] + b4[3];
                    if (oacc) {
                        uint2 old = *p;
                        v0 += bf_lo(old.x); v1 += bf_hi(old.x); v2 += bf_lo(old.y); v3 += bf_hi(old.y);
                    }
                    uint2 o;
                    o.x = pack_bf16x2(v0, v1); o.y = pack_bf16x2(v2, v3);
                    *p = o;
                    if (!SC && a.stats) {
                        float r0 = bf_lo(o.x), r1 = bf_hi(o.x), r2 = bf_lo(o.y), r3 = bf_hi(o.y);
                        s1[n][0] += r0; s1[n][1] += r1; s1[n][2] += r2; s1[n][3] += r3;
                        s2[n][0] = fmaf(r0, r0, s2[n][0]); s2[n][1] = fmaf(r1, r1, s2[n][1]);
                        s2[n][2] = fmaf(r2, r2, s2[n][2]); s2[n][3] = fmaf(r3, r3, s2[n][3]);
                    }
                }
                acc[i][n] = f32x4{0.f, 0.f, 0.f, 0.f};
            }
        }
    }
    if (!SC && a.stats) {
        float* red = (float*)smem;
        __syncthreads();
#pragma unroll
        for (int n = 0; n < NT; ++n)
#pragma unroll
            for (int r = 0; r < 4; ++r) {
                float u = s1[n][r], v = s2[n][r];
#pragma unroll
                for (int m = 1; m < 16; m <<= 1) { u += __shfl_xor(u, m); v += __shfl_xor(v, m); }
                if (j == 0) {
                    int cl = n * 16 + gq * 4 + r;
                    red[(wave * NT * 16 + cl) * 2 + 0] = u;
                    red[(wave * NT * 16 + cl) * 2 + 1] = v;
                }
            }
        __syncthreads();
        if (tid < NT * 16) {
            float u = 0.f, v = 0.f;
#pragma unroll
            for (int w = 0; w < NW; ++w) { u += red[(w * NT * 16 + tid) * 2]; v += red[(w * NT * 16 + tid) * 2 + 1]; }
            int c = nt0 * 16 + tid;
            a.stats[((size_t)blockIdx.x * g.Cout + c) * 2 + 0] = u;
            a.stats[((size_t)blockIdx.x * g.Cout + c) * 2 + 1] = v;
        }
    }
}

constexpr int SMALL_QS = 8;
template <int BZ, int BY, int BX, int OCC, bool BNS = false, int NW = 4>
__global__ void __launch_bounds__(NW * 64, OCC) k_mfma_conv_small(MfmaConvArgs a) {
    constexpr int NTHR = NW * 64;
    constexpr int HZ = BZ + 2, HY = BY + 2, HX = BX + 2, HXP = (HX + 3) / 4 * 4;
    constexpr int TXM = BX < 16 ? BX : 16, TYM = 16 / TXM, RG = BY / TYM;
    constexpr int TILE_B = HZ * HY * HXP * 64;
    constexpr int UNITS = HZ * HY * HX * 4, ITERS = (UNITS + NTHR - 1) / NTHR;
    constexpr int QB = OCC == 1 ? 4 : 2;
    static_assert(BZ * BY * BX == 64, "four m-tiles per tile");
    static_assert(NW == 4 || (NW == 8 && OCC == 1), "eight waves: the one-block-per-CU form only");
    extern __shared__ __attribute__((aligned(16))) char smem[];

    const ConvGeom& g = a.g;
    const int tid = threadIdx.x, wave = tid >> 6, lane = tid & 63, j = lane & 15, gq = lane >> 4, lg = tid & 3;
    const int nt0 = blockIdx.x, NTT = g.Cout / 16, nchunk = g.Cin / 32, C0 = a.src[0].C;
    const int bid = blockIdx.y;
    const int x0 = (bid % a.tiles_x) * BX, y0 = ((bid / a.tiles_x) % a.tiles_y) * BY, z0 = (bid / (a.tiles_x * a.tiles_y)) * BZ;
    const int iz0 = z0 - 1, iy0 = y0 - 1, ix0 = x0 - 1;
    const bf16x8* wp = (const bf16x8*)a.w;

    int mbase[4][3];
#pragma unroll
    for (int i = 0; i < 4; ++i) {
        const int mz = i / RG, my = (i % RG) * TYM + j / TXM, mx = j % TXM;
#pragma unroll
        for (int kx = 0; kx < 3; ++kx) {
            const int hx = mx + kx;
            mbase[i][kx] = ((mz * HY + my) * HXP + hx) * 64 + ((gq ^ (((hx >> 2) & 1) << 1)) << 4);
        }
    }
    int ulds[ITERS];
    unsigned uvox[ITERS], uin = 0;
#pragma unroll
    for (int it = 0; it < ITERS; ++it) {
        const int u = tid + it * NTHR;
        const int hv = u >> 2, hz = hv / (HY * HX), hr = hv % (HY * HX), hy = hr / HX, hx = hr % HX;
        ulds[it] = u < UNITS ? ((hz * HY + hy) * HXP + hx) * 64 + ((lg ^ (((hx >> 2) & 1) << 1)) << 4) : -1;
        uvox[it] = (unsigned)((hz * g.H + hy) * g.W + hx);
        const int gz = iz0 + hz, gy = iy0 + hy, gx = ix0 + hx;
        if (u < UNITS && (unsigned)gz < (unsigned)g.D && (unsigned)gy < (unsigned)g.H && (unsigned)gx < (unsigned)g.W) uin |= 1u << it;
    }
    const long long org = ((long long)iz0 * g.H + iy0) * g.W + ix0;
    f32x4 acc[4];
#pragma unroll
    for (int i = 0; i < 4; ++i) acc[i] = f32x4{0.f, 0.f, 0.f, 0.f};

    for (int q0 = 0; q0 < nchunk; q0 += SMALL_QS) {
        const int nq = nchunk - q0 < SMALL_QS ? nchunk - q0 : SMALL_QS;
        bf16x8 wf[27];
        {
            const int qq = wave < nq ? wave : 0;
            const bf16x8* wq = wp + ((size_t)(q0 + qq) * 27 * NTT + nt0) * 64 + lane;
#pragma unroll
            for (int ks = 0; ks < 27; ++ks) wf[ks] = wq[(size_t)ks * NTT * 64];
        }
        __syncthreads();
#pragma unroll 1
        for (int qb = 0; qb < nq; qb += QB) {
            uint4 R[QB][ITERS];
#pragma unroll
            for (int qq = 0; qq < QB; ++qq) {
                if (qb + qq < nq) {
                    const int c = (q0 + qb + qq) * 32 + lg * 8;
                    const int sidx = (a.nsrc > 1 && c >= C0) ? 1 : 0;
                    const char* sptr = (const char*)(sidx ? a.src[1].ptr : a.src[0].ptr);
                    const int sC = sidx ? a.src[1].C : C0;
                    const char* base = sptr + (org * sC + (c - (sidx ? C0 : 0))) * 2;
                    const unsigned vstride = (unsigned)sC * 2;
#pragma unroll
                    for (int it = 0; it < ITERS; ++it) {
                        R[qq][it] = make_uint4(0u, 0u, 0u, 0u);
                        if ((uin >> it) & 1u) R[qq][it] = *(const uint4*)(base + __umul24(uvox[it], vstride));
                    }
                }
            }
#pragma unroll
            for (int qq = 0; qq < QB; ++qq) {
                if (qb + qq < nq) {
// ... 12 lines not shown
            bf16x8 xbuf[2][4];
#pragma unroll
            for (int i = 0; i < 4; ++i) xbuf[0][i] = *(const bf16x8*)(tile + mbase[i][0]);
#pragma unroll
            for (int ks = 0; ks < 27; ++ks) {
                if (ks + 1 < 27) {
                    const int k1 = ks + 1, toff = ((k1 / 9) * HY + (k1 / 3) % 3) * HXP * 64;
#pragma unroll
                    for (int i = 0; i < 4; ++i) xbuf[k1 & 1][i] = *(const bf16x8*)(tile + mbase[i][k1 % 3] + toff);
                }
                __builtin_amdgcn_sched_barrier(0);
#pragma unroll
                for (int i = 0; i < 4; ++i) acc[i] = __builtin_amdgcn_mfma_f32_16x16x32_bf16(wf[ks], xbuf[ks & 1][i], acc[i], 0, 0, 0);
                __builtin_amdgcn_sched_barrier(0);
                if (more) wf[ks] = wn[(size_t)ks * NTT * 64];
            }
        }
    }

    __syncthreads();
    float* red = (float*)smem;
#pragma unroll
    for (int i = 0; i < 4; ++i) *(f32x4*)(red + ((wave * 4 + i) * 64 + lane) * 4) = acc[i];
    __syncthreads();
    const int mt = wave & 3;
    f32x4 o4 = *(const f32x4*)(red + ((0 * 4 + mt) * 64 + lane) * 4);
#pragma unroll
    for (int v = 1; v < NW; ++v) {
        const f32x4 t = *(const f32x4*)(red + ((v * 4 + mt) * 64 + lane) * 4);
        o4[0] += t[0]; o4[1] += t[1]; o4[2] += t[2]; o4[3] += t[3];
    }
    float s1[4] = {0.f, 0.f, 0.f, 0.f}, s2[4] = {0.f, 0.f, 0.f, 0.f};
    {
        const int c = nt0 * 16 + gq * 4;
        float b4[4] = {0.f, 0.f, 0.f, 0.f};
        if (a.bias) {
#pragma unroll
            for (int r = 0; r < 4; ++r) b4[r] = a.bias[c + r];
        }
        const int d = (a.nout > 1 && c >= a.outC[0]) ? 1 : 0;
        const int cd = c - (d ? a.outC[0] : 0);
        char* obase = (char*)(d ? a.out[1] : a.out[0]);
        const int oC = d ? a.outC[1] : a.outC[0], oacc = d ? a.out_acc[1] : a.out_acc[0];
        const int mz = mt / RG, my = (mt % RG) * TYM + j / TXM, mx = j % TXM;
        const int gz = z0 + mz, gy = y0 + my, gx = x0 + mx;
        if (wave < 4 && gz < a.oD && gy < a.oH && gx < a.oW && obase) {
            const size_t vox = ((size_t)gz * a.oH + gy) * a.oW + gx;
            uint2* p = (uint2*)(obase + (vox * oC + cd) * 2);
            float v0 = o4[0] + b4[0], v1 = o4[1] + b4[1], v2 = o4[2] + b4[2], v3 = o4[3] + b4[3];
            if (oacc) {
                const uint2 old = *p;
                v0 += bf_lo(old.x); v1 += bf_hi(old.x); v2 += bf_lo(old.y); v3 += bf_hi(old.y);
            }
            uint2 o;
            o.x = pack_bf16x2(v0, v1); o.y = pack_bf16x2(v2, v3);
            *p = o;
            const float r0 = bf_lo(o.x), r1 = bf_hi(o.x), r2 = bf_lo(o.y), r3 = bf_hi(o.y);
            if constexpr (BNS) {
                const uint2 ur = *(const uint2*)((const char*)a.bn_u + (vox * a.bn_C + c) * 2);
                const float uu[4] = {bf_lo(ur.x), bf_hi(ur.x), bf_lo(ur.y), bf_hi(ur.y)}, rr[4] = {r0, r1, r2, r3};
#pragma unroll
                for (int r = 0; r < 4; ++r) {
                    const float mean = a.bn_stat[c + r], rstd = a.bn_stat[a.bn_C + c + r];
                    const float dv = rr[r] * act_d(fmaf(uu[r], a.bn_stat[2 * a.bn_C + c + r], a.bn_stat[3 * a.bn_C + c + r]), a.bn_act);
                    s1[r] = dv; s2[r] = dv * ((uu[r] - mean) * rstd);
                }
            } else {
                s1[0] = r0; s1[1] = r1; s1[2] = r2; s1[3] = r3;
                s2[0] = r0 * r0; s2[1] = r1 * r1; s2[2] = r2 * r2; s2[3] = r3 * r3;
            }
        }
    }
    float* const srows = BNS ? a.bn_partial : a.stats;
    if (srows) {
        __syncthreads();
#pragma unroll
        for (int r = 0; r < 4; ++r) {
            float u = s1[r], v = s2[r];
#pragma unroll
            for (int m = 1; m < 16; m <<= 1) { u += __shfl_xor(u, m); v += __shfl_xor(v, m); }
            if (j == 0) { red[(wave * 16 + gq * 4 + r) * 2] = u; red[(wave * 16 + gq * 4 + r) * 2 + 1] = v; }
        }
        __syncthreads();
        if (tid < 16) {
            float u = 0.f, v = 0.f;
#pragma unroll
            for (int w = 0; w < 4; ++w) { u += red[(w * 16 + tid) * 2]; v += red[(w * 16 + tid) * 2 + 1]; }
            srows[((size_t)bid * g.Cout + nt0 * 16 + tid) * 2 + 0] = u;
            srows[((size_t)bid * g.Cout + nt0 * 16 + tid) * 2 + 1] = v;
        }
    }
}

struct ConvFirstArgs {
    ConvGeom g;
    const void* x;
    const float* w;
    const float* bias;
    void* out;
    float* stats;
    int tiles_x, tiles_y, tiles_z;
};
template <int NT>
__global__ void __launch_bounds__(256, 2) k_conv_first_mfma(ConvFirstArgs a) {
    constexpr int BZ = 4, BY = 8, BX = 16, HZ = BZ + 2, HY = BY + 2, HX = BX + 2, NV = HZ * HY * HX;
    constexpr int ITERS = (NV + 255) / 256;
    __shared__ unsigned short tile[NV + 8];
    __shared__ float red[4 * NT * 16 * 2];
    const ConvGeom& g = a.g;
    const int tid = threadIdx.x, wave = tid >> 6, lane = tid & 63, j = lane & 15, gq = lane >> 4;
    const int ntiles = a.tiles_x * a.tiles_y * a.tiles_z;
    const unsigned short* x = (const unsigned short*)a.x;

    bf16x8 wfrag[NT];
#pragma unroll
    for (int n = 0; n < NT; ++n)
#pragma unroll
        for (int e = 0; e < 8; ++e) {
            const int tap = 8 * gq + e;
            wfrag[n][e] = (__bf16)(tap < 27 ? a.w[(n * 16 + j) * 27 + tap] : 0.f);
        }
    int abase[8];
#pragma unroll
    for (int e = 0; e < 8; ++e) {
        const int tap = 8 * gq + e < 27 ? 8 * gq + e : 26;
        abase[e] = ((((tap / 9) + wave) * HY + (tap / 3) % 3) * HX + tap % 3 + j) * 2;
    }
    float b4[NT][4];
#pragma unroll
    for (int n = 0; n < NT; ++n)
#pragma unroll
        for (int r = 0; r < 4; ++r) b4[n][r] = a.bias ? a.bias[n * 16 + gq * 4 + r] : 0.f;
    float s1[NT][4], s2[NT][4];
#pragma unroll
    for (int n = 0; n < NT; ++n)
#pragma unroll
        for (int r = 0; r < 4; ++r) { s1[n][r] = 0.f; s2[n][r] = 0.f; }

    int upk[ITERS];
    unsigned uvox[ITERS];
#pragma unroll
    for (int k = 0; k < ITERS; ++k) {
        const int u = tid + k * 256, hz = u / (HY * HX), hr = u % (HY * HX), hy = hr / HX, hx = hr % HX;
        upk[k] = u < NV ? (hz | (hy << 4) | (hx << 9)) : -1;
        uvox[k] = (unsigned)((hz * g.H + hy) * g.W + hx);
    }
    unsigned short R[ITERS];
    auto prefetch = [&](int t) {
        const int x0 = (t % a.tiles_x) * BX, y0 = ((t / a.tiles_x) % a.tiles_y) * BY, z0 = (t / (a.tiles_x * a.tiles_y)) * BZ;
        const int iz0 = z0 - 1, iy0 = y0 - 1, ix0 = x0 - 1;
        const long long org = ((long long)iz0 * g.H + iy0) * g.W + ix0;
#pragma unroll
        for (int k = 0; k < ITERS; ++k) {
            const int uc = upk[k];
            const int gz = iz0 + (uc & 15), gy = iy0 + ((uc >> 4) & 31), gx = ix0 + ((uc >> 9) & 63);
            R[k] = 0;
            if (uc >= 0 && (unsigned)gz < (unsigned)g.D && (unsigned)gy < (unsigned)g.H && (unsigned)gx < (unsigned)g.W)
                R[k] = x[org + uvox[k]];
        }
    };
    if ((int)blockIdx.x < ntiles) prefetch(blockIdx.x);
    for (int t = blockIdx.x; t < ntiles; t += gridDim.x) {
        __syncthreads();
#pragma unroll
        for (int k = 0; k < ITERS; ++k)
            if (upk[k] >= 0) tile[tid + k * 256] = R[k];
        __syncthreads();
        if (t + (int)gridDim.x < ntiles) prefetch(t + gridDim.x);
        const int x0 = (t % a.tiles_x) * BX, y0 = ((t / a.tiles_x) % a.tiles_y) * BY, z0 = (t / (a.tiles_x * a.tiles_y)) * BZ;
        const int gz = z0 + wave, gx = x0 + j;
#pragma unroll
        for (int i = 0; i < BY; ++i) {
            unsigned d[4];
#pragma unroll
            for (int e = 0; e < 4; ++e) {
                const unsigned lo = *(const unsigned short*)((const char*)tile + abase[2 * e] + i * HX * 2);
                const unsigned hi = *(const unsigned short*)((const char*)tile + abase[2 * e + 1] + i * HX * 2);
                d[e] = lo | (hi << 16);
            }
            const bf16x8 xfrag = __builtin_bit_cast(bf16x8, make_uint4(d[0], d[1], d[2], d[3]));
            const int gy = y0 + i;
            const bool ok = gz < g.D && gy < g.H && gx < g.W;
            const size_t vox = ((size_t)gz * g.H + gy) * g.W + gx;
#pragma unroll
            for (int n = 0; n < NT; ++n) {
                const f32x4 acc = __builtin_amdgcn_mfma_f32_16x16x32_bf16(wfrag[n], xfrag, f32x4{0.f, 0.f, 0.f, 0.f}, 0, 0, 0);
                if (ok) {
                    uint2 o;
                    o.x = pack_bf16x2(acc[0] + b4[n][0], acc[1] + b4[n][1]);
                    o.y = pack_bf16x2(acc[2] + b4[n][2], acc[3] + b4[n][3]);
                    *(uint2*)((char*)a.out + (vox * g.Cout + n * 16 + gq * 4) * 2) = o;
                    const float r0 = bf_lo(o.x), r1 = bf_hi(o.x), r2 = bf_lo(o.y), r3 = bf_hi(o.y);
                    s1[n][0] += r0; s1[n][1] += r1; s1[n][2] += r2; s1[n][3] += r3;
                    s2[n][0] = fmaf(r0, r0, s2[n][0]); s2[n][1] = fmaf(r1, r1, s2[n][1]);
                    s2[n][2] = fmaf(r2, r2, s2[n][2]); s2[n][3] = fmaf(r3, r3, s2[n][3]);
                }
            }
        }
    }
    if (a.stats) {
#pragma unroll
        for (int n = 0; n < NT; ++n)
#pragma unroll
            for (int r = 0; r < 4; ++r) {
                float u = s1[n][r], v = s2[n][r];
#pragma unroll
                for (int m = 1; m < 16; m <<= 1) { u += __shfl_xor(u, m); v += __shfl_xor(v, m); }
                if (j == 0) {
                    const int cl = n * 16 + gq * 4 + r;
                    red[(wave * NT * 16 + cl) * 2 + 0] = u;
                    red[(wave * NT * 16 + cl) * 2 + 1] = v;
                }
            }
        __syncthreads();
        if (tid < NT * 16) {
            float u = 0.f, v = 0.f;
#pragma unroll
            for (int w = 0; w < 4; ++w) { u += red[(w * NT * 16 + tid) * 2]; v += red[(w * NT * 16 + tid) * 2 + 1]; }
            a.stats[((size_t)blockIdx.x * g.Cout + tid) * 2 + 0] = u;
            a.stats[((size_t)blockIdx.x * g.Cout + tid) * 2 + 1] = v;
        }
    }
}

__global__ void __launch_bounds__(256, 2) k_mfma_conv_z(MfmaConvArgs a, ZWork zw) {
    constexpr int BY = 8, BX = 16, HY = BY + 2, HX = BX + 2, HXP = 20, PLANE_B = HY * HXP * 64, RING = 4;
    constexpr int UNITS = HY * HX * 4, ITERS = (UNITS + 255) / 256;
    extern __shared__ __attribute__((aligned(16))) char smem[];
    const ConvGeom& g = a.g;
    const int tid = threadIdx.x, wave = tid >> 6, lane = tid & 63, j = lane & 15, gq = lane >> 4, lg = tid & 3;
    const int nt0 = blockIdx.y, NTT = g.Cout / 16, C0 = a.src[0].C;
    const bf16x8* wp = (const bf16x8*)a.w;

    bf16x8 wf[27];
#pragma unroll
    for (int ks = 0; ks < 27; ++ks) wf[ks] = wp[((size_t)ks * NTT + nt0) * 64 + lane];
    __builtin_amdgcn_s_waitcnt(0x0F70);
    int mbase[2][3];
#pragma unroll
    for (int i = 0; i < 2; ++i)
#pragma unroll
        for (int kx = 0; kx < 3; ++kx) {
            const int hx = j + kx;
            mbase[i][kx] = ((2 * wave + i) * HXP + hx) * 64 + ((gq ^ (((hx >> 2) & 1) << 1)) << 4);
        }
    int ulds[ITERS], uyx[ITERS];
#pragma unroll
    for (int it = 0; it < ITERS; ++it) {
        const int u = tid + it * 256, hv = u >> 2, hy = hv / HX, hx = hv % HX;
        ulds[it] = u < UNITS ? (hy * HXP + hx) * 64 + ((lg ^ (((hx >> 2) & 1) << 1)) << 4) : -1;
        uyx[it] = hy | (hx << 8);
    }
    const int c = lg * 8, sidx = (a.nsrc > 1 && c >= C0) ? 1 : 0;
    const char* sptr = (const char*)(sidx ? a.src[1].ptr : a.src[0].ptr) + (size_t)(c - (sidx ? C0 : 0)) * 2;
    const int sC = sidx ? a.src[1].C : C0;
    const unsigned vstride = (unsigned)sC * 2;

    float s1[4] = {0.f, 0.f, 0.f, 0.f}, s2[4] = {0.f, 0.f, 0.f, 0.f};
    float b4[4] = {0.f, 0.f, 0.f, 0.f};
    const int cch = nt0 * 16 + gq * 4;
    if (a.bias) {
#pragma unroll
        for (int r = 0; r < 4; ++r) b4[r] = a.bias[cch + r];
    }
    const int dsel = (a.nout > 1 && cch >= a.outC[0]) ? 1 : 0;
    const int cd = cch - (dsel ? a.outC[0] : 0);
    char* obase = (char*)(dsel ? a.out[1] : a.out[0]);
    const int oC = dsel ? a.outC[1] : a.outC[0], oacc = dsel ? a.out_acc[1] : a.out_acc[0];
    const unsigned obytes = obase ? (unsigned)((size_t)a.oD * a.oH * a.oW * oC * 2) : 0u;
    const __amdgpu_buffer_rsrc_t orsrc = __builtin_amdgcn_make_buffer_rsrc(obase, 0, (int)obytes, 0x00020000);
    constexpr int OOB = (int)0x80000000;

    const int nitems = zw.cols_x * zw.cols_y * zw.nseg;
    bf16x8 R[ITERS], R2[ITERS];
    const bf16x8 zero8 = __builtin_bit_cast(bf16x8, make_uint4(0u, 0u, 0u, 0u));
    const int ncols = zw.cols_x * zw.cols_y;
    for (int item = xcd_remap(blockIdx.x, gridDim.x); item < nitems; item += gridDim.x) {
        const int seg = item / ncols, col = item % ncols;
        const int x0 = (col % zw.cols_x) * BX, y0 = (col / zw.cols_x) * BY;
        const int zs = seg * zw.zlen, ze = zs + zw.zlen < g.D ? zs + zw.zlen : g.D;
        unsigned umask = 0;
        const char* ubase[ITERS];
#pragma unroll
        for (int it = 0; it < ITERS; ++it) {
            const int gy = y0 - 1 + (uyx[it] & 255), gx = x0 - 1 + (uyx[it] >> 8);
            const bool ok = ulds[it] >= 0 && (unsigned)gy < (unsigned)g.H && (unsigned)gx < (unsigned)g.W;
            if (ok) umask |= 1u << it;
            ubase[it] = sptr + (size_t)(ok ? gy * g.W + gx : 0) * vstride;
        }
        const size_t plane_bytes = (size_t)g.H * g.W * vstride;
        auto prefetch = [&](int pz, bf16x8 (&Rr)[ITERS]) {
            const bool zin = (unsigned)pz < (unsigned)g.D;
            const size_t po = (size_t)(zin ? pz : 0) * plane_bytes;
#pragma unroll
            for (int it = 0; it < ITERS; ++it) {
                const char* ad = ubase[it] + po;
                asm volatile("global_load_dwordx4 %0, %1, off" : "=v"(Rr[it]) : "v"(ad) : "memory");
            }
        };
        static_assert(ITERS == 3, "the vmcnt values below count 3 plane loads per step");
        auto wait_planes = [&](int younger_stores) {
            if (younger_stores == 4) asm volatile("s_waitcnt vmcnt(7)" ::: "memory");
            else if (younger_stores == 2) asm volatile("s_waitcnt vmcnt(5)" ::: "memory");
// ... 13 lines not shown
            auto load_group = [&](int gi, int sl) {
                const int kz = gi / 3, kx = gi % 3;
#pragma unroll
                for (int r = 0; r < 4; ++r)
                    xr[sl][r] = *(const bf16x8*)(smem + mbase[0][kx] + ((SL + kz) & 3) * PLANE_B + r * HXP * 64);
            };
            load_group(0, 0);
#pragma unroll
            for (int gi = 0; gi < 9; ++gi) {
                if (gi + 1 < 9) load_group(gi + 1, (gi + 1) & 1);
                __builtin_amdgcn_sched_barrier(0);
                const int kz = gi / 3, kx = gi % 3;
#pragma unroll
                for (int ky = 0; ky < 3; ++ky)
#pragma unroll
                    for (int i = 0; i < 2; ++i)
                        acc[i] = __builtin_amdgcn_mfma_f32_16x16x32_bf16(wf[(kz * 3 + ky) * 3 + kx], xr[gi & 1][i + ky],
                                                                         (gi == 0 && ky == 0) ? f32x4{0.f, 0.f, 0.f, 0.f} : acc[i], 0, 0, 0);
                __builtin_amdgcn_sched_barrier(0);
            }
#pragma unroll
            for (int i = 0; i < 2; ++i) {
                float v0 = acc[i][0] + b4[0], v1 = acc[i][1] + b4[1], v2 = acc[i][2] + b4[2], v3 = acc[i][3] + b4[3];
                if (oacc && ook[i]) {
                    const uint2 old = *(const uint2*)(obase + ooff[i]);
                    v0 += bf_lo(old.x); v1 += bf_hi(old.x); v2 += bf_lo(old.y); v3 += bf_hi(old.y);
                }
                typedef __attribute__((ext_vector_type(2))) unsigned u32x2;
                u32x2 o;
                o.x = pack_bf16x2(v0, v1); o.y = pack_bf16x2(v2, v3);
                __builtin_amdgcn_raw_buffer_store_b64(o, orsrc, ook[i] ? (int)ooff[i] : OOB, 0, 0);
                if (a.stats && ook[i]) {
                    const float r0 = bf_lo(o.x), r1 = bf_hi(o.x), r2 = bf_lo(o.y), r3 = bf_hi(o.y);
                    s1[0] += r0; s1[1] += r1; s1[2] += r2; s1[3] += r3;
                    s2[0] = fmaf(r0, r0, s2[0]); s2[1] = fmaf(r1, r1, s2[1]); s2[2] = fmaf(r2, r2, s2[2]); s2[3] = fmaf(r3, r3, s2[3]);
                }
                ooff[i] += oplane;
            }
        };

        auto step = [&](int pz, bf16x8 (&Rc)[ITERS], auto par) {
            constexpr int PAR = decltype(par)::value;
            const bool computes = pz >= zs + 2;
            if (computes) {
                if (((pz - 2) & 2) == 0) plane(std::integral_constant<int, PAR>{});
                else plane(std::integral_constant<int, 2 + PAR>{});
            }
            const int slot = (pz + 1) & 3;
            const bool zin = (unsigned)pz < (unsigned)g.D;
            wait_planes(pz >= zs + 3 ? 4 : (computes ? 2 : 0));
#pragma unroll
            for (int it = 0; it < ITERS; ++it)
                if (ulds[it] >= 0) {
                    char* d = smem + slot * PLANE_B + ulds[it];
                    const unsigned dl = (unsigned)(size_t)(__attribute__((address_space(3))) char*)d;
                    asm volatile("ds_write_b128 %0, %1" :: "v"(dl), "v"(Rc[it]) : "memory");
                    if (!(zin && ((umask >> it) & 1u))) *(bf16x8*)d = zero8;
                }
            prefetch(pz + 2 <= ze ? pz + 2 : ze, Rc);
            __syncthreads();
        };
        __syncthreads();
        asm volatile("s_waitcnt vmcnt(0)" ::: "memory");
        const int pe0 = (zs - 1) & ~1;
        prefetch(pe0, R);
        prefetch(pe0 + 1, R2);
        for (int pe = pe0; pe <= ze + 1; pe += 2) {
            step(pe, R, std::integral_constant<int, 0>{});
            if (pe + 1 <= ze + 1) step(pe + 1, R2, std::integral_constant<int, 1>{});
        }
    }
    asm volatile("s_waitcnt vmcnt(0)" ::: "memory");
    if (a.stats) {
        float* red = (float*)smem;
        __syncthreads();
#pragma unroll
        for (int r = 0; r < 4; ++r) {
            float u = s1[r], v = s2[r];
#pragma unroll
            for (int m = 1; m < 16; m <<= 1) { u += __shfl_xor(u, m); v += __shfl_xor(v, m); }
            if (j == 0) { red[(wave * 16 + gq * 4 + r) * 2] = u; red[(wave * 16 + gq * 4 + r) * 2 + 1] = v; }
        }
        __syncthreads();
        if (tid < 16) {
            float u = 0.f, v = 0.f;
#pragma unroll
            for (int w = 0; w < 4; ++w) { u += red[(w * 16 + tid) * 2]; v += red[(w * 16 + tid) * 2 + 1]; }
            a.stats[((size_t)blockIdx.x * g.Cout + nt0 * 16 + tid) * 2 + 0] = u;
            a.stats[((size_t)blockIdx.x * g.Cout + nt0 * 16 + tid) * 2 + 1] = v;
        }
    }
}
static int launch_conv_z(const MfmaConvArgs& a0, hipStream_t s) {
    const ConvGeom& g = a0.g;
    if (sliding_window_off() || g.Cin != 32 || g.Wo < 12 || g.Do < 8 || g.D != g.Do || g.H != g.Ho || g.W != g.Wo) return 0;
    for (int k = 0; k < 2; ++k)
        if (a0.out[k] && (size_t)a0.oD * a0.oH * a0.oW * a0.outC[k] * 2 >= ((size_t)1 << 31)) return 0;
    ZWork zw;
    zw.cols_x = (g.Wo + 15) / 16; zw.cols_y = (g.Ho + 7) / 8;
    const int cols = zw.cols_x * zw.cols_y, gy = g.Cout / 16;
    int want = 512 / gy;
    if (want < 1) want = 1;
    int nseg = (want + cols - 1) / cols;
    if (nseg < 1) nseg = 1;
    int zlen = (g.Do + nseg - 1) / nseg;
    if (zlen < 4) zlen = 4;
    nseg = (g.Do + zlen - 1) / zlen;
    zw.nseg = nseg; zw.zlen = zlen;
    const int items = cols * nseg;
    const int gx = items < want ? items : want;
    constexpr int lds = 4 * 10 * 20 * 64;
    static std::atomic<uint64_t> attr_done{0};
    set_max_lds_once(attr_done, (const void*)k_mfma_conv_z, lds);
    k_mfma_conv_z<<<dim3((unsigned)gx, (unsigned)gy), 256, lds, s>>>(a0, zw);
    return gx;
}

template <int S, int KD, int PAD, int BZ, int BY, int BX, int CK, int NT, bool SC>
static int launch_cfg(const MfmaConvArgs& a0, hipStream_t s) {
    constexpr int NW = ((BZ * BY * BX / 16) % 8 == 0 && BZ * BY * BX >= 256 && (NT > 1 || SC)) ? 8 : 4;
    MfmaConvArgs a = a0;
    a.tiles_x = (a.g.Wo + BX - 1) / BX; a.tiles_y = (a.g.Ho + BY - 1) / BY; a.tiles_z = (a.g.Do + BZ - 1) / BZ;
    constexpr bool SWZ = CK == 32 && S == 1 && KD == 3;
    constexpr int VS = SWZ ? 64 : (CK == 32 ? 96 : 32);
    constexpr int HXr = (BX - 1) * S + KD, HXP = SWZ ? (HXr + 3) / 4 * 4 : HXr;
    constexpr int T = KD * KD * KD, KSTEPS = CK == 32 ? T : (T + 1) / 2;
    constexpr size_t tile_b = (size_t)((BZ - 1) * S + KD) * ((BY - 1) * S + KD) * HXP * VS;
    constexpr size_t lds = tile_b + (KSTEPS * NT <= 32 ? (size_t)KSTEPS * NT * 1024 : 0);
    static_assert(tile_b >= NW * NT * 16 * 2 * 4, "stats scratch must fit the tile buffer");
    static_assert(lds <= 80 * 1024 || (S == 2 && KD == 3 && CK == 32 && lds <= 128 * 1024), "LDS per block");
    static std::atomic<uint64_t> attr_done{0};
    set_max_lds_once(attr_done, (const void*)k_mfma_conv_p<S, KD, PAD, BZ, BY, BX, CK, NT, SC, NW, false>, (int)lds);
    const int tiles = a.tiles_x * a.tiles_y * a.tiles_z, gy = a.g.Cout / (16 * NT);
    constexpr int bpc = (lds <= 40 * 1024 && NW == 4) ? 4 : 2;
    int gx = bpc * 256 / gy;
    if (gx < 1) gx = 1;
    if (gx > tiles) gx = tiles;
    dim3 grid((unsigned)gx, (unsigned)gy);
    if constexpr (NT == 1 && !SC) {
        if (a.g.Cin == CK) {
            static std::atomic<uint64_t> attr4_done{0};
            set_max_lds_once(attr4_done, (const void*)k_mfma_conv_p<S, KD, PAD, BZ, BY, BX, CK, NT, SC, 4, true>, (int)lds);
            k_mfma_conv_p<S, KD, PAD, BZ, BY, BX, CK, NT, SC, 4, true><<<grid, 256, lds, s>>>(a);
            return gx;
        }
    }
    k_mfma_conv_p<S, KD, PAD, BZ, BY, BX, CK, NT, SC, NW, false><<<grid, NW * 64, lds, s>>>(a);
    return gx;
}
template <int S, int KD, int PAD, int BZ, int BY, int BX, int CK, bool SC> static int launch_nt(const MfmaConvArgs& a, hipStream_t s) {
    int ntt = a.g.Cout / 16;
    if constexpr (SC) {
        int tiles = ((a.g.Wo + BX - 1) / BX) * ((a.g.Ho + BY - 1) / BY) * ((a.g.Do + BZ - 1) / BZ);
        int nt = 4;
        if constexpr (BX <= 8) {
            while (nt > 1 && (int64_t)tiles * (ntt / nt) < 256) nt >>= 1;
            if (nt == 1) return launch_cfg<S, KD, PAD, BZ, BY, BX, CK, 1, true>(a, s);
            if (nt == 2) return launch_cfg<S, KD, PAD, BZ, BY, BX, CK, 2, true>(a, s);
        }
        return launch_cfg<S, KD, PAD, BZ, BY, BX, CK, 4, true>(a, s);
    } else {
        int tiles = ((a.g.Wo + BX - 1) / BX) * ((a.g.Ho + BY - 1) / BY) * ((a.g.Do + BZ - 1) / BZ);
        int nt = ntt % 4 == 0 ? 4 : (ntt % 2 == 0 ? 2 : 1);
        constexpr int T = KD * KD * KD, KSTEPS = CK == 32 ? T : (T + 1) / 2;
        while (nt > 1 && KSTEPS * nt > 32) nt >>= 1;
        while (nt > 1 && (int64_t)tiles * (ntt / nt) < 256) nt >>= 1;
        if (CK == 16 && a.g.Cin == 16 && nt == 2 && S == 1 && KD == 3) nt = 1;
        if (nt == 4) return launch_cfg<S, KD, PAD, BZ, BY, BX, CK, 4, false>(a, s);
        if (nt == 2) return launch_cfg<S, KD, PAD, BZ, BY, BX, CK, 2, false>(a, s);
        return launch_cfg<S, KD, PAD, BZ, BY, BX, CK, 1, false>(a, s);
    }
}
// ... 251 lines not shown
```

### unet-studio_amd/csrc/kernels_mfma_conv_z16.hip

```cpp
#include <cstdlib>
#include <type_traits>

#include "mfma_util.h"

namespace unet {

__device__ __attribute__((aligned(16))) unsigned g_z16_zero[4] = {0u, 0u, 0u, 0u};

template <int NT, bool BNS>
__global__ void __launch_bounds__(256, 2) k_mfma_conv_z16(MfmaConvArgs a, ZWork zw) {
    constexpr int BY = 8, BX = 16, HY = BY + 2, HX = BX + 2, PLANE_B = HY * HX * 32;
    constexpr int UNITS = HY * HX * 2, UPW = UNITS / 4, ITERS = 2;
    constexpr int NBUF = 6, PF = 5;
    constexpr int UOFF = NBUF * PLANE_B, UTILE_B = BY * BX * 32;
    static_assert(UTILE_B == 4 * 64 * 16, "one piece per wave");
    static_assert(UPW == 90 && NBUF % 3 == 0 && NBUF >= PF + 1, "unit split / ring");
    extern __shared__ __attribute__((aligned(16))) char smem[];
    const ConvGeom& g = a.g;
    const int tid = threadIdx.x, wave = tid >> 6, lane = tid & 63, j = lane & 15, gq = lane >> 4, h = gq >> 1, lg = lane & 1;
    const int nt0 = blockIdx.y * NT, NTT = g.Cout / 16, C0 = a.src[0].C;
    const bf16x8* wp = (const bf16x8*)a.w;
    const bf16x8 zero8 = __builtin_bit_cast(bf16x8, make_uint4(0u, 0u, 0u, 0u));
    const unsigned lds0 = (unsigned)(size_t)(__attribute__((address_space(3))) char*)smem;

// ... 141 lines not shown
                        }
            const int k = r - 3;
            const bool kin = k >= 0 && zs + k < ze;
#pragma unroll
            for (int i = 0; i < 2; ++i)
#pragma unroll
                for (int n = 0; n < NT; ++n) {
                    const f32x4 d = acc[(PH + 1) % 3][i][n];
                    const bool ok = kin && ook[i] && ohave[n];
                    const int off = ok ? (int)(ooff[i][n] + (unsigned)k * oplane[n]) : OOB;
                    float v0 = d[0] + b4[n][0], v1 = d[1] + b4[n][1], v2 = d[2] + b4[n][2], v3 = d[3] + b4[n][3];
                    typedef __attribute__((ext_vector_type(2))) unsigned u32x2;
                    if (oacc[n]) {
                        const u32x2 old = __builtin_amdgcn_raw_buffer_load_b64(orsrc[n], off, 0, 0);
                        v0 += bf_lo(old.x); v1 += bf_hi(old.x); v2 += bf_lo(old.y); v3 += bf_hi(old.y);
                    }
                    u32x2 o;
                    o.x = pack_bf16x2(v0, v1); o.y = pack_bf16x2(v2, v3);
                    __builtin_amdgcn_raw_buffer_store_b64(o, orsrc[n], off, 0, 0);
                    const float r0 = ok ? bf_lo(o.x) : 0.f, r1 = ok ? bf_hi(o.x) : 0.f, r2 = ok ? bf_lo(o.y) : 0.f, r3 = ok ? bf_hi(o.y) : 0.f;
                    if constexpr (BNS) {
                        const uint2 uu = *(const uint2*)(smem + UOFF + BQ * UTILE_B + ((2 * wave + i) * BX + j) * 32 + gq * 8);
                        const float uf[4] = {bf_lo(uu.x), bf_hi(uu.x), bf_lo(uu.y), bf_hi(uu.y)}, rr[4] = {r0, r1, r2, r3};
#pragma unroll
                        for (int c = 0; c < 4; ++c) {
                            const float dv = rr[c] * act_d(fmaf(uf[c], bsc[c], bsh[c]), a.bn_act);
                            s1[n][c] += dv;
                            s2[n][c] = fmaf(dv, (uf[c] - bmean[c]) * brstd[c], s2[n][c]);
                        }
                    } else {
                        s1[n][0] += r0; s1[n][1] += r1; s1[n][2] += r2; s1[n][3] += r3;
                        s2[n][0] = fmaf(r0, r0, s2[n][0]); s2[n][1] = fmaf(r1, r1, s2[n][1]);
                        s2[n][2] = fmaf(r2, r2, s2[n][2]); s2[n][3] = fmaf(r3, r3, s2[n][3]);
                    }
                }
        };
        auto step = [&](int r, auto phc, auto slc) {
            constexpr int SL = decltype(slc)::value;
            static_assert(PF == 5, "vmcnt below = (P + 2) PF - P, P = 2 pieces (3 with the raw-tensor tile)");
            if constexpr (BNS) asm volatile("s_waitcnt vmcnt(22)\n\ts_barrier" ::: "memory");
            else asm volatile("s_waitcnt vmcnt(18)\n\ts_barrier" ::: "memory");
            dma(r - 1 + PF, (SL + PF) % NBUF);
            compute(r, phc, slc);
        };
        asm volatile("s_waitcnt vmcnt(0)\n\ts_barrier" ::: "memory");
#pragma unroll
        for (int r = 0; r < PF; ++r) {
            dma(r, r);
#pragma unroll
            for (int i = 0; i < 2 * NT; ++i) {
                typedef __attribute__((ext_vector_type(2))) unsigned u32x2;
                __builtin_amdgcn_raw_buffer_store_b64(u32x2{0u, 0u}, orsrc[0], OOB + 8 * (r * 2 * NT + i), 0, 0);
            }
        }
        for (int r = 1; r <= rlast; r += 6) {
            step(r, std::integral_constant<int, 1>{}, std::integral_constant<int, 0>{});
            if (r + 1 > rlast) break;
            step(r + 1, std::integral_constant<int, 2>{}, std::integral_constant<int, 1>{});
            if (r + 2 > rlast) break;
            step(r + 2, std::integral_constant<int, 0>{}, std::integral_constant<int, 2>{});
            if (r + 3 > rlast) break;
            step(r + 3, std::integral_constant<int, 1>{}, std::integral_constant<int, 3>{});
            if (r + 4 > rlast) break;
            step(r + 4, std::integral_constant<int, 2>{}, std::integral_constant<int, 4>{});
            if (r + 5 > rlast) break;
            step(r + 5, std::integral_constant<int, 0>{}, std::integral_constant<int, 5>{});
        }
    }
    asm volatile("s_waitcnt vmcnt(0)\n\ts_barrier" ::: "memory");
    float* const srows = BNS ? a.bn_partial : a.stats;
    const int srowC = BNS ? a.bn_C : g.Cout;
    if (srows) {
        float* red = (float*)smem;
#pragma unroll
        for (int n = 0; n < NT; ++n)
#pragma unroll
            for (int r = 0; r < 4; ++r) {
                float u = s1[n][r], v = s2[n][r];
#pragma unroll
                for (int m = 1; m < 16; m <<= 1) { u += __shfl_xor(u, m); v += __shfl_xor(v, m); }
                if (j == 0) { red[((wave * NT + n) * 16 + gq * 4 + r) * 2] = u; red[((wave * NT + n) * 16 + gq * 4 + r) * 2 + 1] = v; }
            }
        __syncthreads();
        if (tid < NT * 16) {
            float u = 0.f, v = 0.f;
#pragma unroll
            for (int w = 0; w < 4; ++w) { u += red[((w * NT) * 16 + tid) * 2]; v += red[((w * NT) * 16 + tid) * 2 + 1]; }
            srows[((size_t)blockIdx.x * srowC + nt0 * 16 + tid) * 2 + 0] = u;
            srows[((size_t)blockIdx.x * srowC + nt0 * 16 + tid) * 2 + 1] = v;
        }
    }
}

__global__ void __launch_bounds__(256, 2) k_mfma_conv_z32(MfmaConvArgs a, ZWork zw) {
    constexpr int BY = 8, BX = 16, HY = BY + 2, HX = BX + 2, PLANE_B = HY * HX * 64;
    constexpr int UNITS = HY * HX * 4, UPW = UNITS / 4, ITERS = 3;
    constexpr int NBUF = 6, PF = 5;
    static_assert(UPW == 180 && UPW % 4 == 0 && NBUF % 3 == 0 && NBUF >= PF + 1, "unit split / ring");
    extern __shared__ __attribute__((aligned(16))) char smem[];
    const ConvGeom& g = a.g;
    const int tid = threadIdx.x, wave = tid >> 6, lane = tid & 63, j = lane & 15, gq = lane >> 4;
    const int nt0 = blockIdx.y, NTT = g.Cout / 16, C0 = a.src[0].C;
    const bf16x8* wp = (const bf16x8*)a.w;
    const unsigned lds0 = (unsigned)(size_t)(__attribute__((address_space(3))) char*)smem;

    bf16x8 wf[27];
#pragma unroll
    for (int ks = 0; ks < 27; ++ks) wf[ks] = wp[((size_t)ks * NTT + nt0) * 64 + lane];
    int mb[4][3];
#pragma unroll
    for (int R = 0; R < 4; ++R)
#pragma unroll
        for (int kx = 0; kx < 3; ++kx) {
            const int hv = (2 * wave + R) * HX + j + kx;
            mb[R][kx] = hv * 64 + ((gq ^ (((hv >> 2) & 1) << 1)) << 4);
        }
    int uyx[ITERS];
    bool uact[ITERS];
    unsigned upiece[ITERS];
#pragma unroll
    for (int it = 0; it < ITERS; ++it) {
        const int u = wave * UPW + it * 64 + lane, hv = u >> 2, hy = hv / HX, hx = hv % HX;
        uact[it] = it * 64 + lane < UPW;
        uyx[it] = hy | (hx << 8) | ((((u & 3) ^ (((hv >> 2) & 1) << 1))) << 16);
        upiece[it] = (unsigned)__builtin_amdgcn_readfirstlane((wave * UPW + it * 64) * 16);
    }

    float s1[4], s2[4], b4[4];
    const int cch = nt0 * 16 + gq * 4;
#pragma unroll
    for (int r = 0; r < 4; ++r) { s1[r] = 0.f; s2[r] = 0.f; b4[r] = a.bias ? a.bias[cch + r] : 0.f; }
    const int dsel = (a.nout > 1 && nt0 * 16 >= a.outC[0]) ? 1 : 0;
    char* ob = (char*)(dsel ? a.out[1] : a.out[0]);
    const int oC = dsel ? a.outC[1] : a.outC[0], oacc = dsel ? a.out_acc[1] : a.out_acc[0], cd = cch - (dsel ? a.outC[0] : 0);
    const bool ohave = ob != nullptr;
    const __amdgpu_buffer_rsrc_t orsrc = __builtin_amdgcn_make_buffer_rsrc(ob, 0, ob ? (int)((size_t)a.oD * a.oH * a.oW * oC * 2) : 0, 0x00020000);
    constexpr int OOB = (int)0x80000000;

    const int nitems = zw.cols_x * zw.cols_y * zw.nseg, ncols = zw.cols_x * zw.cols_y;
    for (int item = xcd_remap(blockIdx.x, gridDim.x); item < nitems; item += gridDim.x) {
        const int seg = item / ncols, col = item % ncols;
        const int x0 = (col % zw.cols_x) * BX, y0 = (col / zw.cols_x) * BY;
        const int zs = seg * zw.zlen, ze = zs + zw.zlen < g.D ? zs + zw.zlen : g.D;
        bool uok[ITERS];
        const char* ubase[ITERS];
        unsigned uvs[ITERS];
#pragma unroll
        for (int it = 0; it < ITERS; ++it) {
            const int gy = y0 - 1 + (uyx[it] & 255), gx = x0 - 1 + ((uyx[it] >> 8) & 255), c = (uyx[it] >> 16) * 8;
            const int sidx = (a.nsrc > 1 && c >= C0) ? 1 : 0;
            uok[it] = uact[it] && (unsigned)gy < (unsigned)g.H && (unsigned)gx < (unsigned)g.W;
            uvs[it] = (unsigned)(sidx ? a.src[1].C : C0) * 2;
            ubase[it] = (const char*)(sidx ? a.src[1].ptr : a.src[0].ptr) + (size_t)(c - (sidx ? C0 : 0)) * 2 + (size_t)(uok[it] ? gy * g.W + gx : 0) * uvs[it];
        }
        const size_t hw = (size_t)g.H * g.W;
        const int rlast = (ze - zs) + 2;
        auto dma = [&](int r, int slot) {
            const int pz = zs - 1 + r;
            const bool zin = (unsigned)pz < (unsigned)g.D && r < rlast;
#pragma unroll
            for (int it = 0; it < ITERS; ++it) {
                const char* src = (zin && uok[it]) ? ubase[it] + (size_t)pz * hw * uvs[it] : (const char*)g_z16_zero;
                const unsigned dst = lds0 + (unsigned)slot * PLANE_B + upiece[it];
                unsigned keep;
                if (it < 2 || uact[it])
                    asm volatile("s_mov_b32 %0, m0\n\ts_mov_b32 m0, %2\n\ts_nop 0\n\tglobal_load_lds_dwordx4 %1, off\n\ts_mov_b32 m0, %0"
                                 : "=&s"(keep) : "v"(src), "s"(dst) : "memory");
            }
        };
        const int ox = x0 + j;
        bool ook[2];
        unsigned ooff[2];
// ... 13 lines not shown
        auto compute = [&](int r, auto phc, auto slc) {
            constexpr int PH = decltype(phc)::value, BQ = decltype(slc)::value;
            bf16x8 xr[4][3];
#pragma unroll
            for (int kx = 0; kx < 3; ++kx)
#pragma unroll
                for (int R = 0; R < 4; ++R) xr[R][kx] = *(const bf16x8*)(smem + BQ * PLANE_B + mb[R][kx]);
            __builtin_amdgcn_sched_barrier(0);
#pragma unroll
            for (int kx = 0; kx < 3; ++kx)
#pragma unroll
                for (int ky = 0; ky < 3; ++ky)
#pragma unroll
                    for (int kz = 0; kz < 3; ++kz)
#pragma unroll
                        for (int i = 0; i < 2; ++i) {
                            f32x4& d = acc[(PH - kz + 3) % 3][i];
                            d = __builtin_amdgcn_mfma_f32_16x16x32_bf16(wf[kz * 9 + ky * 3 + kx], xr[i + ky][kx],
                                                                        (kz == 0 && kx == 0 && ky == 0) ? f32x4{0.f, 0.f, 0.f, 0.f} : d, 0, 0, 0);
                        }
            const int k = r - 3;
            const bool kin = k >= 0 && zs + k < ze;
#pragma unroll
            for (int i = 0; i < 2; ++i) {
                const f32x4 d = acc[(PH + 1) % 3][i];
                const bool ok = kin && ook[i] && ohave;
                const int off = ok ? (int)(ooff[i] + (unsigned)k * oplane) : OOB;
                float v0 = d[0] + b4[0], v1 = d[1] + b4[1], v2 = d[2] + b4[2], v3 = d[3] + b4[3];
                typedef __attribute__((ext_vector_type(2))) unsigned u32x2;
                if (oacc) {
                    const u32x2 old = __builtin_amdgcn_raw_buffer_load_b64(orsrc, off, 0, 0);
                    v0 += bf_lo(old.x); v1 += bf_hi(old.x); v2 += bf_lo(old.y); v3 += bf_hi(old.y);
                }
                u32x2 o;
                o.x = pack_bf16x2(v0, v1); o.y = pack_bf16x2(v2, v3);
                __builtin_amdgcn_raw_buffer_store_b64(o, orsrc, off, 0, 0);
                const float r0 = ok ? bf_lo(o.x) : 0.f, r1 = ok ? bf_hi(o.x) : 0.f, r2 = ok ? bf_lo(o.y) : 0.f, r3 = ok ? bf_hi(o.y) : 0.f;
                s1[0] += r0; s1[1] += r1; s1[2] += r2; s1[3] += r3;
                s2[0] = fmaf(r0, r0, s2[0]); s2[1] = fmaf(r1, r1, s2[1]); s2[2] = fmaf(r2, r2, s2[2]); s2[3] = fmaf(r3, r3, s2[3]);
            }
        };
        auto step = [&](int r, auto phc, auto slc) {
            constexpr int SL = decltype(slc)::value;
            static_assert(PF == 5, "vmcnt below = 5 PF - 3");
            asm volatile("s_waitcnt vmcnt(22)\n\ts_barrier" ::: "memory");
            dma(r - 1 + PF, (SL + PF) % NBUF);
            compute(r, phc, slc);
        };
        asm volatile("s_waitcnt vmcnt(0)\n\ts_barrier" ::: "memory");
#pragma unroll
        for (int r = 0; r < PF; ++r) {
            dma(r, r);
#pragma unroll
            for (int i = 0; i < 2; ++i) {
                typedef __attribute__((ext_vector_type(2))) unsigned u32x2;
                __builtin_amdgcn_raw_buffer_store_b64(u32x2{0u, 0u}, orsrc, OOB + 8 * (r * 2 + i), 0, 0);
            }
        }
        for (int r = 1; r <= rlast; r += 6) {
            step(r, std::integral_constant<int, 1>{}, std::integral_constant<int, 0>{});
            if (r + 1 > rlast) break;
            step(r + 1, std::integral_constant<int, 2>{}, std::integral_constant<int, 1>{});
            if (r + 2 > rlast) break;
            step(r + 2, std::integral_constant<int, 0>{}, std::integral_constant<int, 2>{});
            if (r + 3 > rlast) break;
            step(r + 3, std::integral_constant<int, 1>{}, std::integral_constant<int, 3>{});
            if (r + 4 > rlast) break;
            step(r + 4, std::integral_constant<int, 2>{}, std::integral_constant<int, 4>{});
            if (r + 5 > rlast) break;
            step(r + 5, std::integral_constant<int, 0>{}, std::integral_constant<int, 5>{});
        }
    }
    asm volatile("s_waitcnt vmcnt(0)\n\ts_barrier" ::: "memory");
    if (a.stats) {
        float* red = (float*)smem;
#pragma unroll
        for (int r = 0; r < 4; ++r) {
            float u = s1[r], v = s2[r];
#pragma unroll
            for (int m = 1; m < 16; m <<= 1) { u += __shfl_xor(u, m); v += __shfl_xor(v, m); }
            if (j == 0) { red[(wave * 16 + gq * 4 + r) * 2] = u; red[(wave * 16 + gq * 4 + r) * 2 + 1] = v; }
        }
        __syncthreads();
        if (tid < 16) {
            float u = 0.f, v = 0.f;
#pragma unroll
            for (int w = 0; w < 4; ++w) { u += red[(w * 16 + tid) * 2]; v += red[(w * 16 + tid) * 2 + 1]; }
            a.stats[((size_t)blockIdx.x * g.Cout + nt0 * 16 + tid) * 2 + 0] = u;
            a.stats[((size_t)blockIdx.x * g.Cout + nt0 * 16 + tid) * 2 + 1] = v;
        }
    }
}

int launch_conv_z32(const MfmaConvArgs& a0, hipStream_t s) {
    const ConvGeom& g = a0.g;
    if (sliding_window_off() || g.Cin != 32 || g.ks != 3 || g.stride != 1 || g.Wo < 12 || g.Do < 8 || g.D != g.Do || g.H != g.Ho || g.W != g.Wo) return 0;
    for (int k = 0; k < 2; ++k)
        if (a0.out[k] && (size_t)a0.oD * a0.oH * a0.oW * a0.outC[k] * 2 >= ((size_t)1 << 31)) return 0;
    if (a0.nout > 1 && a0.outC[0] % 16) return 0;
    for (int k = 0; k < a0.nsrc; ++k) if (a0.src[k].C % 8) return 0;
    ZWork zw;
    zw.cols_x = (g.Wo + 15) / 16; zw.cols_y = (g.Ho + 7) / 8;
    const int cols = zw.cols_x * zw.cols_y, gy = g.Cout / 16;
    int want = 512 / gy;
    if (want < 1) want = 1;
    int nseg = (want + cols - 1) / cols;
    if (nseg < 1) nseg = 1;
    int zlen = (g.Do + nseg - 1) / nseg;
    if (zlen < 4) zlen = 4;
    nseg = (g.Do + zlen - 1) / zlen;
    zw.nseg = nseg; zw.zlen = zlen;
    const int items = cols * nseg;
    const int gx = items < want ? items : want;
    constexpr int lds = 6 * 10 * 18 * 64;
    static std::atomic<uint64_t> attr_done{0};
    set_max_lds_once(attr_done, (const void*)k_mfma_conv_z32, lds);
    k_mfma_conv_z32<<<dim3((unsigned)gx, (unsigned)gy), 256, lds, s>>>(a0, zw);
    return gx;
}

bool conv_z16_applies(const MfmaConvArgs& a0) {
    const ConvGeom& g = a0.g;
    if (sliding_window_off() || g.Cin != 16 || g.ks != 3 || g.stride != 1 || g.Wo < 12 || g.Do < 8 || g.D != g.Do || g.H != g.Ho || g.W != g.Wo) return false;
    if (g.Cout != 16 && g.Cout != 32) return false;
    for (int k = 0; k < 2; ++k)
        if (a0.out[k] && (size_t)a0.oD * a0.oH * a0.oW * a0.outC[k] * 2 >= ((size_t)1 << 31)) return false;
    if (a0.nout > 1 && a0.outC[0] % 16) return false;
    return true;
}
int launch_conv_z16(const MfmaConvArgs& a0, hipStream_t s) {
    const ConvGeom& g = a0.g;
    if (!conv_z16_applies(a0)) return 0;
    ZWork zw;
    zw.cols_x = (g.Wo + 15) / 16; zw.cols_y = (g.Ho + 7) / 8;
    const int cols = zw.cols_x * zw.cols_y;
    const int gy = g.Cout / 16;
    const int want = 512 / gy;
    int nseg = (want + cols - 1) / cols;
    if (nseg < 1) nseg = 1;
    int zlen = (g.Do + nseg - 1) / nseg;
    if (zlen < 4) zlen = 4;
    nseg = (g.Do + zlen - 1) / zlen;
    zw.nseg = nseg; zw.zlen = zlen;
    const int items = cols * nseg;
    const int gx = items < want ? items : want;
    constexpr int lds = 6 * 10 * 18 * 32;
    if (a0.bn_partial) k_mfma_conv_z16<1, true><<<dim3((unsigned)gx, (unsigned)gy), 256, lds + 6 * 8 * 16 * 32, s>>>(a0, zw);
    else k_mfma_conv_z16<1, false><<<dim3((unsigned)gx, (unsigned)gy), 256, lds, s>>>(a0, zw);
    return gx;
}

}
```

### unet-studio_amd/csrc/kernels_mfma_s2.hip

```cpp
#include <cstdlib>
#include <type_traits>

#include "mfma_util.h"

namespace unet {

__device__ __attribute__((aligned(16))) unsigned g_s2_zero[4] = {0u, 0u, 0u, 0u};

struct S2ScatterArgs {
    const void* src;
    int srcC;
    int cD, cH, cW;
    const void* w;
    const float* bias;
    void* out;
    int outC;
    int fD, fH, fW;
    int ntt;
    const void* bn_u = nullptr;
    const float* bn_stat = nullptr;
    float* bn_partial = nullptr;
    int bn_act = 0, bn_C = 0;
    int cols_x, cols_y, nseg, zlen;
};
// ... 448 lines not shown
#pragma unroll
        for (int i = 0; i < NR; ++i) { accC[i] = f32x4{0.f, 0.f, 0.f, 0.f}; accN[i] = f32x4{0.f, 0.f, 0.f, 0.f}; }

        auto compute = [&](int r, auto slc) {
            constexpr int SL = decltype(slc)::value, PAR = SL & 1;
            const char* pin = smem + SL * PLANE_B;
            constexpr bool FIN = KS == 3 ? PAR == 0 : PAR == 1;
#pragma unroll
            for (int i = 0; i < NR; ++i)
#pragma unroll
                for (int s = 0; s < NKS; ++s) {
                    const bf16x8 x = *(const bf16x8*)(pin + mb[s] + i * 2 * HXV * VB);
                    if constexpr (KS == 3 && PAR == 0) {
                        accC[i] = __builtin_amdgcn_mfma_f32_16x16x32_bf16(wf[2][s], x, accC[i], 0, 0, 0);
                        accN[i] = __builtin_amdgcn_mfma_f32_16x16x32_bf16(wf[0][s], x, s == 0 ? f32x4{0.f, 0.f, 0.f, 0.f} : accN[i], 0, 0, 0);
                    } else if constexpr (KS == 3) {
                        accC[i] = __builtin_amdgcn_mfma_f32_16x16x32_bf16(wf[1][s], x, accC[i], 0, 0, 0);
                    } else if constexpr (PAR == 0) {
                        accC[i] = __builtin_amdgcn_mfma_f32_16x16x32_bf16(wf[0][s], x, s == 0 ? f32x4{0.f, 0.f, 0.f, 0.f} : accC[i], 0, 0, 0);
                    } else {
                        accC[i] = __builtin_amdgcn_mfma_f32_16x16x32_bf16(wf[1][s], x, accC[i], 0, 0, 0);
                    }
                    if constexpr (NR * NKS > 18) { if (s == NKS - 1) __builtin_amdgcn_sched_barrier(0); }
                }
            const int k = KS == 3 ? (r >> 1) - 1 : (r >> 1);
#pragma unroll
            for (int i = 0; i < NR; ++i) {
                if constexpr (FIN) {
                    const f32x4 d = accC[i];
                    const bool ok = k >= 0 && k < len && ook[i];
                    const int off = ok ? (int)(ooff[i] + (unsigned)k * oplane) : OOB;
                    u32x2 o;
                    o.x = pack_bf16x2(d[0] + b4[0], d[1] + b4[1]); o.y = pack_bf16x2(d[2] + b4[2], d[3] + b4[3]);
                    __builtin_amdgcn_raw_buffer_store_b64(o, orsrc, off, 0, 0);
                    const float r0 = ok ? bf_lo(o.x) : 0.f, r1 = ok ? bf_hi(o.x) : 0.f, r2 = ok ? bf_lo(o.y) : 0.f, r3 = ok ? bf_hi(o.y) : 0.f;
                    s1[0] += r0; s1[1] += r1; s1[2] += r2; s1[3] += r3;
                    s2[0] = fmaf(r0, r0, s2[0]); s2[1] = fmaf(r1, r1, s2[1]); s2[2] = fmaf(r2, r2, s2[2]); s2[3] = fmaf(r3, r3, s2[3]);
                    if constexpr (KS == 3) accC[i] = accN[i];
                } else {
                    __builtin_amdgcn_raw_buffer_store_b64(u32x2{0u, 0u}, orsrc, OOB + 8 * (i + 1), 0, 0);
                }
            }
        };
        auto step = [&](int r, auto slc) {
            constexpr int SL = decltype(slc)::value;
            asm volatile("s_waitcnt vmcnt(%0)\n\ts_barrier" :: "n"(WAITN) : "memory");
            dma(r + PF, (SL + PF) % NBUF);
            compute(r, slc);
        };
        asm volatile("s_waitcnt vmcnt(0)\n\ts_barrier" ::: "memory");
#pragma unroll
        for (int r = 0; r < PF; ++r) {
            dma(r, r);
#pragma unroll
            for (int i = 0; i < S; ++i) __builtin_amdgcn_raw_buffer_store_b64(u32x2{0u, 0u}, orsrc, OOB + 64 + 8 * (r * S + i), 0, 0);
        }
        for (int r = 0; r <= rlast; r += NBUF) {
            step(r, std::integral_constant<int, 0>{});
            if (r + 1 > rlast) break;
            step(r + 1, std::integral_constant<int, 1>{});
            if (r + 2 > rlast) break;
            step(r + 2, std::integral_constant<int, 2>{});
            if (r + 3 > rlast) break;
            step(r + 3, std::integral_constant<int, 3>{});
            if constexpr (NBUF == 6) {
                if (r + 4 > rlast) break;
                step(r + 4, std::integral_constant<int, 4>{});
                if (r + 5 > rlast) break;
                step(r + 5, std::integral_constant<int, 5>{});
            }
        }
    }
    asm volatile("s_waitcnt vmcnt(0)\n\ts_barrier" ::: "memory");
    if (a.stats) {
        float* red = (float*)smem;
#pragma unroll
        for (int r = 0; r < 4; ++r) {
            float u = s1[r], v = s2[r];
#pragma unroll
            for (int m = 1; m < 16; m <<= 1) { u += __shfl_xor(u, m); v += __shfl_xor(v, m); }
            if (j == 0) { red[(wave * 16 + gq * 4 + r) * 2] = u; red[(wave * 16 + gq * 4 + r) * 2 + 1] = v; }
        }
        __syncthreads();
        if (tid < WM * 16) {
            const int m = tid >> 4, c = tid & 15;
            float u = 0.f, v = 0.f;
#pragma unroll
            for (int g = 0; g < 4 / WM; ++g) { u += red[((g * WM + m) * 16 + c) * 2]; v += red[((g * WM + m) * 16 + c) * 2 + 1]; }
            a.stats[((size_t)blockIdx.x * a.outC + (blockIdx.y * WM + m) * 16 + c) * 2 + 0] = u;
            a.stats[((size_t)blockIdx.x * a.outC + (blockIdx.y * WM + m) * 16 + c) * 2 + 1] = v;
        }
    }
}

static void s2_gather_work(S2GatherArgs& a, int gy, int* gx) {
    a.cols_x = (a.cW + 15) / 16; a.cols_y = (a.cH + 3) / 4;
    const int cols = a.cols_x * a.cols_y;
    int want = 512 / gy;
    if (want < 1) want = 1;
    int nseg = (want + cols - 1) / cols;
    if (nseg < 1) nseg = 1;
    int zlen = (a.cD + nseg - 1) / nseg;
    if (zlen < 2) zlen = 2;
    if (zlen > a.cD) zlen = a.cD;
    a.nseg = (a.cD + zlen - 1) / zlen; a.zlen = zlen;
    const int items = cols * a.nseg;
    *gx = items < want ? items : want;
}
template <int KS, int CIN, int WM>
static void launch_gather_t(const S2GatherArgs& a, int gx, int gy, hipStream_t s) {
    constexpr int HY = 8 + (KS == 3 ? 1 : 0), HXV = (KS == 3 ? 17 : 16) + 16, UNITS = HY * HXV * (CIN / 8), UPW = (UNITS + 3) / 4;
    constexpr int PLANE_B = (4 * UPW * 16 + 255) / 256 * 256, lds = (CIN == 16 ? 6 : 4) * PLANE_B;
    static_assert(lds <= 80 * 1024, "two blocks per CU");
    static std::atomic<uint64_t> attr_done{0};
    set_max_lds_once(attr_done, (const void*)k_s2_gather<KS, CIN, WM>, lds);
    k_s2_gather<KS, CIN, WM><<<dim3((unsigned)gx, (unsigned)gy), 256, lds, s>>>(a);
}
template <int KS>
static void launch_gather(const S2GatherArgs& a, int cin, int wm, int gx, int gy, hipStream_t s) {
    if (cin == 16) {
        if (wm == 4) launch_gather_t<KS, 16, 4>(a, gx, gy, s); else if (wm == 2) launch_gather_t<KS, 16, 2>(a, gx, gy, s); else launch_gather_t<KS, 16, 1>(a, gx, gy, s);
    } else {
        if constexpr (KS == 2) { if (wm == 4) { launch_gather_t<KS, 32, 4>(a, gx, gy, s); return; } }
        if (wm == 2) launch_gather_t<KS, 32, 2>(a, gx, gy, s); else launch_gather_t<KS, 32, 1>(a, gx, gy, s);
    }
}
static int s2_wm(int rows, int ks, int cin) {
    const int t = rows / 16;
    int wm = t % 4 == 0 ? 4 : (t % 2 == 0 ? 2 : 1);
    if (ks == 3 && cin == 32 && wm == 4) wm = 2;
    return wm;
}

int launch_s2_conv_fwd(const ConvGeom& g, const SrcDesc* src, int nsrc, const void* w_mfma, const float* bias, void* out, float* stats_partial,
                       hipStream_t s) {
    if (s2_off() || g.ks != 3 || g.stride != 2 || (g.Cin != 16 && g.Cin != 32) || g.Cout % 16 || g.Wo < 16 || g.Do < 4) return 0;
    int csum = 0;
    for (int k = 0; k < nsrc; ++k) { if (src[k].C % 8 || src[k].scale || src[k].act) return 0; csum += src[k].C; }
    if (csum != g.Cin || (size_t)g.Do * g.Ho * g.Wo * g.Cout * 2 >= ((size_t)1 << 31)) return 0;
    S2GatherArgs a;
    a.nsrc = nsrc; a.src[0] = src[0]; if (nsrc > 1) a.src[1] = src[1];
    a.fD = g.D; a.fH = g.H; a.fW = g.W;
    a.w = w_mfma; a.bias = bias; a.out = out; a.outC = g.Cout; a.cD = g.Do; a.cH = g.Ho; a.cW = g.Wo; a.stats = stats_partial;
    const int wm = s2_wm(g.Cout, 3, g.Cin), gy = g.Cout / (16 * wm);
    int gx = 0;
    s2_gather_work(a, gy, &gx);
    launch_gather<3>(a, g.Cin, wm, gx, gy, s);
    return gx;
}
bool launch_s2_convt_dgrad(const ConvGeom& g, const void* dy, const void* w_mfma_dgrad, const DstGrad* dst, int ndst, hipStream_t s) {
    if (s2_off() || ndst != 1 || !dst[0].ptr || dst[0].accumulate || dst[0].C != g.Cin) return false;
    if ((g.Cout != 16 && g.Cout != 32) || g.Cin % 16 || g.W < 16 || g.D < 4) return false;
    if ((size_t)g.D * g.H * g.W * g.Cin * 2 >= ((size_t)1 << 31)) return false;
    S2GatherArgs a;
    a.nsrc = 1; a.src[0].ptr = dy; a.src[0].C = g.Cout;
    a.fD = g.Do; a.fH = g.Ho; a.fW = g.Wo;
    a.w = w_mfma_dgrad; a.bias = nullptr; a.out = dst[0].ptr; a.outC = g.Cin; a.cD = g.D; a.cH = g.H; a.cW = g.W; a.stats = nullptr;
    const int wm = s2_wm(g.Cin, 2, g.Cout), gy = g.Cin / (16 * wm);
    int gx = 0;
    s2_gather_work(a, gy, &gx);
    launch_gather<2>(a, g.Cout, wm, gx, gy, s);
    return true;
}

}
```

Measured before the change: 789.5 million.

## Accumulate BN conv statistics via fixed-point atomics into shared row buckets

Conv kernels no longer write per-block partial sums and squares to a large partial buffer. They now atomically add fixed-point (hi/lo int64) sums into a small set of 32 row buckets, and a fused finalize/apply kernel reads these buckets directly. The bucket buffer is zeroed inside the input pack kernel when possible, which avoids a separate memset. This is meant to cut the separate partial-reduction pass and its memory traffic, at the cost of global atomics contention and deterministic fixed-point overflow handling via a NaN flag.

```diff
diff --git a/unet-studio_amd/csrc/device_util.h b/unet-studio_amd/csrc/device_util.h
--- a/unet-studio_amd/csrc/device_util.h
+++ b/unet-studio_amd/csrc/device_util.h
@@ -148,6 +148,63 @@
     }
 }
 
+__device__ __forceinline__ void stat_rows_add(float* rows_, int C, int row, int c0, int nch, float a, float b) {
+    long long* const rows = (long long*)rows_;
+    const int l = threadIdx.x & 63;
+    for (int h = 0; h < nch; h += 32) {
+        const int from = h + (((l >> 5) << 4) | (l & 15));
+        const float ua = __shfl(a, from), ub = __shfl(b, from);
+        if (l >= 2 * (nch - h)) continue;
+        const float v = (l & 16) ? ub : ua;
+        if (!(fabsf(v) <= STAT_ROWS_MAX)) {
+            __hip_atomic_fetch_or((unsigned long long*)(rows + (size_t)STAT_ROWS_R * 4 * C), 1ull, __ATOMIC_RELAXED, __HIP_MEMORY_SCOPE_AGENT);
+            continue;
+        }
+        const double d = (double)v, hi = rint(d * 256.0), lo = rint((d - hi * (1.0 / 256.0)) * 0x1p52);
+        long long* const cell = rows + (size_t)(row % STAT_ROWS_R) * 4 * C + 2 * (c0 + h) + l;
+        __hip_atomic_fetch_add(cell, (long long)hi, __ATOMIC_RELAXED, __HIP_MEMORY_SCOPE_AGENT);
+        __hip_atomic_fetch_add(cell + 2 * C, (long long)lo, __ATOMIC_RELAXED, __HIP_MEMORY_SCOPE_AGENT);
+    }
+}
+__device__ __forceinline__ void stat_rows_read(const float* rows_, int C, double* sa, double* sb, long long* stage) {
+    const long long* const rows = (const long long*)rows_;
+    const int NP = 2 * C, RG = NP >= 256 ? 1 : 256 / NP;
+    for (int idx = threadIdx.x; idx < NP * RG; idx += 256) {
+        const int p = idx % NP, rg = idx / NP;
+        long long H = 0, W = 0;
+        for (int r0 = rg; r0 < STAT_ROWS_R; r0 += 8 * RG) {
+            long long h[8], w[8];
+#pragma unroll
+            for (int k = 0; k < 8; ++k) {
+                const int r = r0 + k * RG;
+                h[k] = r < STAT_ROWS_R ? rows[(size_t)r * 4 * C + p] : 0;
+                w[k] = r < STAT_ROWS_R ? rows[(size_t)r * 4 * C + NP + p] : 0;
+            }
+#pragma unroll
+            for (int k = 0; k < 8; ++k) { H += h[k]; W += w[k]; }
+        }
+        if (RG > 1) { stage[rg * NP + p] = H; stage[512 + rg * NP + p] = W; }
+        else {
+            const int c = (p >> 5) * 16 + (p & 15);
+            ((p & 16) ? sb : sa)[c] = (double)H * (1.0 / 256.0) + (double)W * 0x1p-52;
+        }
+    }
+    if (RG > 1) {
+        __syncthreads();
+        if (threadIdx.x < NP) {
+            const int p = threadIdx.x, c = (p >> 5) * 16 + (p & 15);
+            long long H = 0, W = 0;
+            for (int q = 0; q < RG; ++q) { H += stage[q * NP + p]; W += stage[512 + q * NP + p]; }
+            ((p & 16) ? sb : sa)[c] = (double)H * (1.0 / 256.0) + (double)W * 0x1p-52;
+        }
+    }
+    __syncthreads();
+    if (rows[(size_t)STAT_ROWS_R * 4 * C] != 0) {
+        for (int c = threadIdx.x; c < C; c += 256) { sa[c] = __builtin_nan(""); sb[c] = __builtin_nan(""); }
+        __syncthreads();
+    }
+}
+
 static inline unsigned cdiv64(int64_t a, int64_t b) { return (unsigned)((a + b - 1) / b); }
 
 }
diff --git a/unet-studio_amd/csrc/engine.cpp b/unet-studio_amd/csrc/engine.cpp
--- a/unet-studio_amd/csrc/engine.cpp
+++ b/unet-studio_amd/csrc/engine.cpp
@@ -91,6 +91,8 @@
     std::vector<WgradReduceJob> wz_jobs;
     WgradReduceJob* wz_jobs_dev = nullptr;
     size_t partial_off = 0, partial_bytes = 0;
+    std::vector<size_t> n_rows;
+    size_t rows_off = 0, rows_bytes = 0;
     size_t ws_bytes = 0;
     size_t loss_bytes = 0;
     std::vector<int64_t> p_off;
@@ -233,6 +235,14 @@
         }
         partial_bytes = pmax ? pmax : 256;
         partial_off = take(partial_bytes);
+        n_rows.assign(g.norms.size(), SIZE_MAX);
+        rows_off = off;
+        for (size_t i = 0; i < g.ops.size(); ++i) {
+            const Op& op = g.ops[i];
+            if (op.kind != OP_CONV || g.tensors[op.dst].norm < 0 || !stat_rows_ok(dtype, op.cout)) continue;
+            if (conv[i].mfma_fwd() || conv[i].fwd == Fwd::first_mfma) n_rows[g.tensors[op.dst].norm] = take(stat_rows_bytes(op.cout));
+        }
+        rows_bytes = off - rows_off;
         size_t wmax = 0, hmax = 0;
         for (size_t i = 0; i < g.ops.size(); ++i) {
             const Op& op = g.ops[i];
@@ -332,9 +342,17 @@
 namespace {
 
 void norm_fwd_passes(int dtype, const void* raw, int C, int64_t S, float* partial, int rows, bool dbl, bool eval, const float* gamma,
-                     const float* beta, double eps, float* stat, float* rm, float* rv, int act, void* act_out, hipStream_t s) {
+                     const float* beta, double eps, float* stat, float* rm, float* rv, int act, void* act_out, hipStream_t s,
+                     bool shared = false) {
     if (eval) launch_norm_eval(C, gamma, beta, rm, rv, eps, stat, s);
-    else {
+    else if (shared) {
+        const int g8 = C / 8;
+        if (act_out && (g8 & (g8 - 1)) == 0) {
+            launch_norm_rows_apply(partial, C, S, gamma, beta, eps, stat, rm, rv, 0.1, raw, act, act_out, s);
+            return;
+        }
+        launch_norm_finalize_rows(partial, C, S, gamma, beta, eps, stat, rm, rv, 0.1, s);
+    } else {
         if (!rows) {
             launch_stats_partial(dtype, raw, C, S, partial, s);
             rows = stats_blocks(S);
@@ -379,6 +397,7 @@
     float* stat(int n) const { return (float*)(ws + p.n_stat[n]); }
     float* coef(int n) const { return (float*)(ws + p.n_coef[n]); }
     float* partial() const { return (float*)(ws + p.partial_off); }
+    float* stat_rows(int n) const { return p.n_rows[n] == SIZE_MAX ? nullptr : (float*)(ws + p.n_rows[n]); }
 
     SrcDesc raw_src(int t) const {
         const Tensor& T = p.g.tensors[t];
@@ -405,7 +424,10 @@
         mode &= 1;
         std::vector<int> fused_blocks(g.norms.size(), 0);
         std::vector<char> fused_dbl(g.norms.size(), 0);
+        std::vector<char> fused_shared(g.norms.size(), 0);
         std::vector<char> fused_done(g.norms.size(), 0);
+        const bool clear_in_pack = p.rows_bytes && !g.ops.empty() && g.ops[0].kind == OP_PACK_INPUT;
+        if (p.rows_bytes && !clear_in_pack) HIP_OK(hipMemsetAsync(ws + p.rows_off, 0, p.rows_bytes, s));
         bool packed = false, pack_pending = false, pack2_pending = false;
         if (p.jobs_dev && packs_current) { packed = true; deep_on = true; }
         else if (p.jobs_dev) {
@@ -446,7 +468,8 @@
             ProfScope ps((int)i, (op.kind == OP_CONV || op.kind == OP_CONVT) ? UNET_PROF_CONV_FWD : op.kind == OP_NORM ? UNET_PROF_NORM_FWD : UNET_PROF_OTHER, s);
             switch (op.kind) {
                 case OP_PACK_INPUT:
-                    launch_pack_input(p.dtype, x, tptr(op.dst), g.in_c, g.tensors[op.dst].voxels(), s);
+                    launch_pack_input(p.dtype, x, tptr(op.dst), g.in_c, g.tensors[op.dst].voxels(), s,
+                                      (clear_in_pack && i == 0) ? ws + p.rows_off : nullptr, p.rows_bytes);
                     break;
                 case OP_CONV:
                 case OP_CONVT: {
@@ -472,7 +495,8 @@
                         else launch_convt_fwd_direct(p.dtype, cg, sd, op.nsrc, wf, params[op.bias], tptr(op.dst), s);
                         break;
                     }
-                    float* const part = want_stats ? partial() : nullptr;
+                    float* const srows = want_stats ? stat_rows(T.norm) : nullptr;
+                    float* const part = !want_stats ? nullptr : (c.mfma_fwd() || c.fwd == Fwd::first_mfma) ? srows : partial();
                     int rows = 0;
                     switch (c.fwd) {
                         case Fwd::deep:
@@ -521,7 +545,8 @@
                             break;
                     }
                     if (want_stats) {
-                        fused_blocks[T.norm] = rows;
+                        fused_blocks[T.norm] = part ? rows : 0;
+                        fused_shared[T.norm] = part && part == srows && rows > 0;
                         fused_dbl[T.norm] = c.fwd == Fwd::first_f32_mfma || c.fwd == Fwd::f32_mfma;
                     }
                     break;
@@ -530,10 +555,10 @@
                     const Norm& n = g.norms[op.norm];
                     const Tensor& T = g.tensors[n.tensor];
                     if (fused_done[op.norm]) break;
-                    norm_fwd_passes(p.dtype, tptr(n.tensor), n.C, T.voxels(), partial(), fused_blocks[op.norm], fused_dbl[op.norm] != 0,
-                                    n.batch && mode == 0, params[n.gamma], params[n.beta], n.eps, stat(op.norm),
-                                    n.batch ? buffers[n.buffer] : nullptr, n.batch ? buffers[n.buffer + 1] : nullptr, T.act,
-                                    p.a_off[n.tensor] != SIZE_MAX ? ws + p.a_off[n.tensor] : nullptr, s);
+                    norm_fwd_passes(p.dtype, tptr(n.tensor), n.C, T.voxels(), fused_shared[op.norm] ? stat_rows(op.norm) : partial(),
+                                    fused_blocks[op.norm], fused_dbl[op.norm] != 0, n.batch && mode == 0, params[n.gamma], params[n.beta], n.eps,
+                                    stat(op.norm), n.batch ? buffers[n.buffer] : nullptr, n.batch ? buffers[n.buffer + 1] : nullptr, T.act,
+                                    p.a_off[n.tensor] != SIZE_MAX ? ws + p.a_off[n.tensor] : nullptr, s, fused_shared[op.norm] != 0);
                     break;
                 }
                 case OP_MATERIALIZE: {
@@ -1420,11 +1445,18 @@
         if (c.mfma_fwd()) {
             void* wm = (char*)scratch + L.pack;
             launch_mfma_pack_conv_w(w, wm, nullptr, g, s);
-            int rows = launch_mfma_conv_fwd(g, &sd, 1, wm, b, y, stats ? part : nullptr, s);
-            if (stats) launch_stats_sum(part, rows, cout, stats, s);
+            const bool shared = stats && stat_rows_ok(dtype, cout);
+            if (shared) HIP_OK(hipMemsetAsync(part, 0, stat_rows_bytes(cout), s));
+            launch_mfma_conv_fwd(g, &sd, 1, wm, b, y, shared ? part : nullptr, s);
+            if (shared) launch_stats_sum_rows(part, cout, stats, s);
+            else if (stats) {
+                launch_stats_partial(dtype, y, cout, So, part, s);
+                launch_stats_sum(part, stats_blocks(So), cout, stats, s);
+            }
         } else if (c.fwd == Fwd::first_mfma) {
-            int rows = launch_conv_first_mfma(g, &sd, w, b, y, stats ? part : nullptr, s);
-            if (stats) launch_stats_sum(part, rows, cout, stats, s);
+            if (stats) HIP_OK(hipMemsetAsync(part, 0, stat_rows_bytes(cout), s));
+            launch_conv_first_mfma(g, &sd, w, b, y, stats ? part : nullptr, s);
+            if (stats) launch_stats_sum_rows(part, cout, stats, s);
         } else {
             op_pack(w, cin, cout, ks * ks * ks, false, scratch, &wf, &wd, s);
             if (c.fwd == Fwd::f32_mfma) {
@@ -1499,9 +1531,11 @@
         launch_mfma_pack_conv_w(w, wm, nullptr, g, s);
         const DeepNormFwd nf = {gamma, beta, eps, stat, rm, rv, momentum, use_running ? 1 : 0, act, y_act};
         if (!(c.fwd == Fwd::deep && launch_deep_conv_fwd(g, sd, nsrc, wm, b, y, &nf, op_deep(), s))) {
-            const int rows = launch_mfma_conv_fwd(g, sd, nsrc, wm, b, y, use_running ? nullptr : part, s);
-            norm_fwd_passes(UNET_DTYPE_BF16, y, cout, (int64_t)g.Do * g.Ho * g.Wo, part, rows, false, use_running != 0, gamma, beta, eps,
-                            stat, rm, rv, act, y_act, s);
+            const bool shared = !use_running && stat_rows_ok(UNET_DTYPE_BF16, cout);
+            if (shared) HIP_OK(hipMemsetAsync(part, 0, stat_rows_bytes(cout), s));
+            const int rows = launch_mfma_conv_fwd(g, sd, nsrc, wm, b, y, shared ? part : nullptr, s);
+            norm_fwd_passes(UNET_DTYPE_BF16, y, cout, (int64_t)g.Do * g.Ho * g.Wo, part, shared ? rows : 0, false, use_running != 0, gamma, beta,
+                            eps, stat, rm, rv, act, y_act, s, shared);
         }
     })
 }
diff --git a/unet-studio_amd/csrc/kernels.h b/unet-studio_amd/csrc/kernels.h
--- a/unet-studio_amd/csrc/kernels.h
+++ b/unet-studio_amd/csrc/kernels.h
@@ -40,7 +40,7 @@
 void launch_pack_conv_w(const float* w, float* w_fwd, float* w_dgrad, int Cin, int Cout, int k3, hipStream_t s);
 void launch_pack_convt_w(const float* w, float* w_fwd, float* w_dgrad, int Cin, int Cout, hipStream_t s);
 
-void launch_pack_input(int dtype, const float* x_ncdhw, void* y, int C, int64_t S, hipStream_t s);
+void launch_pack_input(int dtype, const float* x_ncdhw, void* y, int C, int64_t S, hipStream_t s, void* zero = nullptr, size_t zero_bytes = 0);
 void launch_export(int dtype, SrcDesc src, float* y_ncdhw, int64_t S, hipStream_t s);
 void launch_import_grad(int dtype, const float* g_ncdhw, void* g, int C, int64_t S, int accumulate, hipStream_t s);
 
@@ -63,6 +63,15 @@
 void launch_norm_finalize(const float* partial, int nblk, int C, int64_t S, const float* gamma, const float* beta, double eps,
                           float* stat, float* running_mean, float* running_var, double momentum, hipStream_t s, bool dbl = false);
 void launch_stats_sum(const float* partial, int nblk, int C, float* out, hipStream_t s, bool dbl = false);
+constexpr int STAT_ROWS_R = 32;
+constexpr float STAT_ROWS_MAX = 1099511627776.f;
+static inline size_t stat_rows_bytes(int C) { return ((size_t)STAT_ROWS_R * 4 * C + 2) * 8; }
+static inline bool stat_rows_ok(int dtype, int C) { return dtype == 1 && C % 16 == 0 && C <= 512; }
+void launch_norm_finalize_rows(const float* rows, int C, int64_t S, const float* gamma, const float* beta, double eps, float* stat,
+                               float* running_mean, float* running_var, double momentum, hipStream_t s);
+void launch_norm_rows_apply(const float* rows, int C, int64_t S, const float* gamma, const float* beta, double eps, float* stat,
+                            float* running_mean, float* running_var, double momentum, const void* raw, int act, void* out, hipStream_t s);
+void launch_stats_sum_rows(const float* rows, int C, float* out, hipStream_t s);
 void launch_norm_eval(int C, const float* gamma, const float* beta, const float* rm, const float* rv, double eps, float* stat,
                       hipStream_t s);
 
diff --git a/unet-studio_amd/csrc/kernels_elem.hip b/unet-studio_amd/csrc/kernels_elem.hip
--- a/unet-studio_amd/csrc/kernels_elem.hip
+++ b/unet-studio_amd/csrc/kernels_elem.hip
@@ -2,14 +2,16 @@
 
 namespace unet {
 
-template <typename T> __global__ void k_pack_input(const float* __restrict__ x, T* __restrict__ y, int C, int64_t S) {
+template <typename T> __global__ void k_pack_input(const float* __restrict__ x, T* __restrict__ y, int C, int64_t S, uint4* __restrict__ zero16,
+                                                   int64_t n16) {
     int64_t i = (int64_t)blockIdx.x * 256 + threadIdx.x;
+    for (int64_t k = i; k < n16; k += (int64_t)gridDim.x * 256) zero16[k] = make_uint4(0u, 0u, 0u, 0u);
     if (i >= S * C) return;
     int c = (int)(i % C); int64_t v = i / C;
     st<T>(y, i, x[(int64_t)c * S + v]);
 }
-void launch_pack_input(int dtype, const float* x, void* y, int C, int64_t S, hipStream_t s) {
-    UNET_DISPATCH(dtype, (k_pack_input<T><<<cdiv64(S * C, 256), 256, 0, s>>>(x, (T*)y, C, S)));
+void launch_pack_input(int dtype, const float* x, void* y, int C, int64_t S, hipStream_t s, void* zero, size_t zero_bytes) {
+    UNET_DISPATCH(dtype, (k_pack_input<T><<<cdiv64(S * C, 256), 256, 0, s>>>(x, (T*)y, C, S, (uint4*)zero, (int64_t)(zero ? zero_bytes / 16 : 0))));
 }
 
 template <typename T> __global__ void k_export(SrcDesc src, float* __restrict__ y, int64_t S) {
@@ -675,6 +677,88 @@
     return true;
 }
 
+__device__ __forceinline__ void rows_finalize(const float* __restrict__ rows, int C, int64_t S, const float* __restrict__ gamma,
+                                              const float* __restrict__ beta, double eps, float* __restrict__ stat, float* rm, float* rv,
+                                              double momentum, double* sa, double* sb, long long* stage, float* s_sc, float* s_sh) {
+    stat_rows_read(rows, C, sa, sb, stage);
+    for (int c = threadIdx.x; c < C; c += 256) {
+        const double mean = sa[c] / (double)S;
+        double var = sb[c] / (double)S - mean * mean;
+        if (var < 0.0) var = 0.0;
+        const double rstd = 1.0 / sqrt(var + eps), sc = (double)gamma[c] * rstd;
+        s_sc[c] = (float)sc; s_sh[c] = (float)((double)beta[c] - mean * sc);
+        if (blockIdx.x == 0) {
+            stat[c] = (float)mean; stat[C + c] = (float)rstd; stat[2 * C + c] = s_sc[c]; stat[3 * C + c] = s_sh[c];
+            if (rm) {
+                rm[c] = (float)((1.0 - momentum) * rm[c] + momentum * mean);
+                rv[c] = (float)((1.0 - momentum) * rv[c] + momentum * (S > 1 ? var * (double)S / (double)(S - 1) : var));
+            }
+        }
+    }
+    __syncthreads();
+}
+__global__ void __launch_bounds__(256) k_norm_finalize_rows(const float* __restrict__ rows, int C, int64_t S, const float* __restrict__ gamma,
+                                                            const float* __restrict__ beta, double eps, float* __restrict__ stat, float* rm,
+                                                            float* rv, double momentum) {
+    __shared__ double sa[FUSED_MAX_C], sb[FUSED_MAX_C];
+    __shared__ long long stage[1024];
+    __shared__ float s_sc[FUSED_MAX_C], s_sh[FUSED_MAX_C];
+    rows_finalize(rows, C, S, gamma, beta, eps, stat, rm, rv, momentum, sa, sb, stage, s_sc, s_sh);
+}
+void launch_norm_finalize_rows(const float* rows, int C, int64_t S, const float* gamma, const float* beta, double eps, float* stat,
+                               float* rm, float* rv, double momentum, hipStream_t s) {
+    k_norm_finalize_rows<<<1, 256, 0, s>>>(rows, C, S, gamma, beta, eps, stat, rm, rv, momentum);
+}
+__global__ void __launch_bounds__(256) k_norm_rows_apply8g(const float* __restrict__ rows, int C, int64_t S, int64_t VPB,
+                                                           const float* __restrict__ gamma, const float* __restrict__ beta, double eps,
+                                                           float* __restrict__ stat, float* rm, float* rv, double momentum,
+                                                           const uint4* __restrict__ in, int act, uint4* __restrict__ out) {
+    __shared__ double sa[FUSED_MAX_C], sb[FUSED_MAX_C];
+    __shared__ long long stage[1024];
+    __shared__ float s_sc[FUSED_MAX_C], s_sh[FUSED_MAX_C];
+    rows_finalize(rows, C, S, gamma, beta, eps, stat, rm, rv, momentum, sa, sb, stage, s_sc, s_sh);
+    const int G8 = C / 8, NV = 256 / G8, grp = threadIdx.x % G8, lane = threadIdx.x / G8, c0 = grp * 8;
+    const int64_t v0 = (int64_t)blockIdx.x * VPB, v1 = v0 + VPB < S ? v0 + VPB : S;
+    float sc[8], sh[8];
+#pragma unroll
+    for (int e = 0; e < 8; ++e) { sc[e] = s_sc[c0 + e]; sh[e] = s_sh[c0 + e]; }
+    auto one = [&](uint4 v) {
+        unsigned w[4] = {v.x, v.y, v.z, v.w};
+#pragma unroll
+        for (int e = 0; e < 4; ++e) {
+            float lo = act_f(fmaf(__uint_as_float(w[e] << 16), sc[2 * e], sh[2 * e]), act);
+            float hi = act_f(fmaf(__uint_as_float(w[e] & 0xffff0000u), sc[2 * e + 1], sh[2 * e + 1]), act);
+            w[e] = (unsigned)__bfloat16_as_ushort(__float2bfloat16(lo)) | ((unsigned)__bfloat16_as_ushort(__float2bfloat16(hi)) << 16);
+        }
+        return make_uint4(w[0], w[1], w[2], w[3]);
+    };
+    int64_t v = v0 + lane;
+    for (; v + 3 * NV < v1; v += 4 * NV) {
+        uint4 r[4];
+#pragma unroll
+        for (int j = 0; j < 4; ++j) r[j] = in[(v + j * NV) * G8 + grp];
+#pragma unroll
+        for (int j = 0; j < 4; ++j) out[(v + j * NV) * G8 + grp] = one(r[j]);
+    }
+    for (; v < v1; v += NV) out[v * G8 + grp] = one(in[v * G8 + grp]);
+}
+void launch_norm_rows_apply(const float* rows, int C, int64_t S, const float* gamma, const float* beta, double eps, float* stat, float* rm,
+                            float* rv, double momentum, const void* raw, int act, void* out, hipStream_t s) {
+    const int64_t nv4 = 4 * (256 / (C / 8));
+    int64_t vpb = S * C >= ((int64_t)1 << 22) ? (S + 4095) / 4096 : (S + 255) / 256;
+    if (vpb < nv4) vpb = nv4;
+    vpb = (vpb + nv4 - 1) / nv4 * nv4;
+    k_norm_rows_apply8g<<<cdiv64(S, vpb), 256, 0, s>>>(rows, C, S, vpb, gamma, beta, eps, stat, rm, rv, momentum, (const uint4*)raw, act,
+                                                       (uint4*)out);
+}
+__global__ void __launch_bounds__(256) k_stats_sum_rows(const float* __restrict__ rows, int C, float* __restrict__ out) {
+    __shared__ double sa[FUSED_MAX_C], sb[FUSED_MAX_C];
+    __shared__ long long stage[1024];
+    stat_rows_read(rows, C, sa, sb, stage);
+    for (int c = threadIdx.x; c < C; c += 256) { out[c * 2] = (float)sa[c]; out[c * 2 + 1] = (float)sb[c]; }
+}
+void launch_stats_sum_rows(const float* rows, int C, float* out, hipStream_t s) { k_stats_sum_rows<<<1, 256, 0, s>>>(rows, C, out); }
+
 void launch_materialize(int dtype, const SrcDesc* src, int nsrc, void* out, int64_t S, hipStream_t s) {
     Src2 a;
     a.n = nsrc; a.s[0] = src[0]; if (nsrc > 1) a.s[1] = src[1];
diff --git a/unet-studio_amd/csrc/kernels_mfma_conv.hip b/unet-studio_amd/csrc/kernels_mfma_conv.hip
--- a/unet-studio_amd/csrc/kernels_mfma_conv.hip
+++ b/unet-studio_amd/csrc/kernels_mfma_conv.hip
@@ -439,13 +439,13 @@
                 }
             }
         __syncthreads();
-        if (tid < NT * 16) {
+        if (tid < 64) {
             float u = 0.f, v = 0.f;
-#pragma unroll
-            for (int w = 0; w < NW; ++w) { u += red[(w * NT * 16 + tid) * 2]; v += red[(w * NT * 16 + tid) * 2 + 1]; }
-            int c = nt0 * 16 + tid;
-            a.stats[((size_t)blockIdx.x * g.Cout + c) * 2 + 0] = u;
-            a.stats[((size_t)blockIdx.x * g.Cout + c) * 2 + 1] = v;
+            if (tid < NT * 16) {
+#pragma unroll
+                for (int w = 0; w < NW; ++w) { u += red[(w * NT * 16 + tid) * 2]; v += red[(w * NT * 16 + tid) * 2 + 1]; }
+            }
+            stat_rows_add(a.stats, g.Cout, blockIdx.x, nt0 * 16, NT * 16, u, v);
         }
     }
 }
@@ -624,12 +624,18 @@
             if (j == 0) { red[(wave * 16 + gq * 4 + r) * 2] = u; red[(wave * 16 + gq * 4 + r) * 2 + 1] = v; }
         }
         __syncthreads();
-        if (tid < 16) {
+        if (tid < 64) {
             float u = 0.f, v = 0.f;
-#pragma unroll
-            for (int w = 0; w < 4; ++w) { u += red[(w * 16 + tid) * 2]; v += red[(w * 16 + tid) * 2 + 1]; }
-            srows[((size_t)bid * g.Cout + nt0 * 16 + tid) * 2 + 0] = u;
-            srows[((size_t)bid * g.Cout + nt0 * 16 + tid) * 2 + 1] = v;
+            if (tid < 16) {
+#pragma unroll
+                for (int w = 0; w < 4; ++w) { u += red[(w * 16 + tid) * 2]; v += red[(w * 16 + tid) * 2 + 1]; }
+            }
+            if constexpr (BNS) {
+                if (tid < 16) {
+                    srows[((size_t)bid * g.Cout + nt0 * 16 + tid) * 2 + 0] = u;
+                    srows[((size_t)bid * g.Cout + nt0 * 16 + tid) * 2 + 1] = v;
+                }
+            } else stat_rows_add(srows, g.Cout, bid, nt0 * 16, 16, u, v);
         }
     }
 }
@@ -755,12 +761,13 @@
                 }
             }
         __syncthreads();
-        if (tid < NT * 16) {
+        if (tid < 64) {
             float u = 0.f, v = 0.f;
-#pragma unroll
-            for (int w = 0; w < 4; ++w) { u += red[(w * NT * 16 + tid) * 2]; v += red[(w * NT * 16 + tid) * 2 + 1]; }
-            a.stats[((size_t)blockIdx.x * g.Cout + tid) * 2 + 0] = u;
-            a.stats[((size_t)blockIdx.x * g.Cout + tid) * 2 + 1] = v;
+            if (tid < NT * 16) {
+#pragma unroll
+                for (int w = 0; w < 4; ++w) { u += red[(w * NT * 16 + tid) * 2]; v += red[(w * NT * 16 + tid) * 2 + 1]; }
+            }
+            stat_rows_add(a.stats, g.Cout, blockIdx.x, 0, NT * 16, u, v);
         }
     }
 }
@@ -940,12 +947,13 @@
             if (j == 0) { red[(wave * 16 + gq * 4 + r) * 2] = u; red[(wave * 16 + gq * 4 + r) * 2 + 1] = v; }
         }
         __syncthreads();
-        if (tid < 16) {
+        if (tid < 64) {
             float u = 0.f, v = 0.f;
-#pragma unroll
-            for (int w = 0; w < 4; ++w) { u += red[(w * 16 + tid) * 2]; v += red[(w * 16 + tid) * 2 + 1]; }
-            a.stats[((size_t)blockIdx.x * g.Cout + nt0 * 16 + tid) * 2 + 0] = u;
-            a.stats[((size_t)blockIdx.x * g.Cout + nt0 * 16 + tid) * 2 + 1] = v;
+            if (tid < 16) {
+#pragma unroll
+                for (int w = 0; w < 4; ++w) { u += red[(w * 16 + tid) * 2]; v += red[(w * 16 + tid) * 2 + 1]; }
+            }
+            stat_rows_add(a.stats, g.Cout, blockIdx.x, nt0 * 16, 16, u, v);
         }
     }
 }
diff --git a/unet-studio_amd/csrc/kernels_mfma_conv_z16.hip b/unet-studio_amd/csrc/kernels_mfma_conv_z16.hip
--- a/unet-studio_amd/csrc/kernels_mfma_conv_z16.hip
+++ b/unet-studio_amd/csrc/kernels_mfma_conv_z16.hip
@@ -247,12 +247,18 @@
                 if (j == 0) { red[((wave * NT + n) * 16 + gq * 4 + r) * 2] = u; red[((wave * NT + n) * 16 + gq * 4 + r) * 2 + 1] = v; }
             }
         __syncthreads();
-        if (tid < NT * 16) {
+        if (tid < 64) {
             float u = 0.f, v = 0.f;
-#pragma unroll
-            for (int w = 0; w < 4; ++w) { u += red[((w * NT) * 16 + tid) * 2]; v += red[((w * NT) * 16 + tid) * 2 + 1]; }
-            srows[((size_t)blockIdx.x * srowC + nt0 * 16 + tid) * 2 + 0] = u;
-            srows[((size_t)blockIdx.x * srowC + nt0 * 16 + tid) * 2 + 1] = v;
+            if (tid < NT * 16) {
+#pragma unroll
+                for (int w = 0; w < 4; ++w) { u += red[((w * NT) * 16 + tid) * 2]; v += red[((w * NT) * 16 + tid) * 2 + 1]; }
+            }
+            if constexpr (BNS) {
+                if (tid < NT * 16) {
+                    srows[((size_t)blockIdx.x * srowC + nt0 * 16 + tid) * 2 + 0] = u;
+                    srows[((size_t)blockIdx.x * srowC + nt0 * 16 + tid) * 2 + 1] = v;
+                }
+            } else stat_rows_add(srows, srowC, blockIdx.x, nt0 * 16, NT * 16, u, v);
         }
     }
 }
@@ -432,12 +438,13 @@
             if (j == 0) { red[(wave * 16 + gq * 4 + r) * 2] = u; red[(wave * 16 + gq * 4 + r) * 2 + 1] = v; }
         }
         __syncthreads();
-        if (tid < 16) {
+        if (tid < 64) {
             float u = 0.f, v = 0.f;
-#pragma unroll
-            for (int w = 0; w < 4; ++w) { u += red[(w * 16 + tid) * 2]; v += red[(w * 16 + tid) * 2 + 1]; }
-            a.stats[((size_t)blockIdx.x * g.Cout + nt0 * 16 + tid) * 2 + 0] = u;
-            a.stats[((size_t)blockIdx.x * g.Cout + nt0 * 16 + tid) * 2 + 1] = v;
+            if (tid < 16) {
+#pragma unroll
+                for (int w = 0; w < 4; ++w) { u += red[(w * 16 + tid) * 2]; v += red[(w * 16 + tid) * 2 + 1]; }
+            }
+            stat_rows_add(a.stats, g.Cout, blockIdx.x, nt0 * 16, 16, u, v);
         }
     }
 }
diff --git a/unet-studio_amd/csrc/kernels_mfma_s2.hip b/unet-studio_amd/csrc/kernels_mfma_s2.hip
--- a/unet-studio_amd/csrc/kernels_mfma_s2.hip
+++ b/unet-studio_amd/csrc/kernels_mfma_s2.hip
@@ -554,13 +554,14 @@
             if (j == 0) { red[(wave * 16 + gq * 4 + r) * 2] = u; red[(wave * 16 + gq * 4 + r) * 2 + 1] = v; }
         }
         __syncthreads();
-        if (tid < WM * 16) {
-            const int m = tid >> 4, c = tid & 15;
+        if (tid < 64) {
             float u = 0.f, v = 0.f;
-#pragma unroll
-            for (int g = 0; g < 4 / WM; ++g) { u += red[((g * WM + m) * 16 + c) * 2]; v += red[((g * WM + m) * 16 + c) * 2 + 1]; }
-            a.stats[((size_t)blockIdx.x * a.outC + (blockIdx.y * WM + m) * 16 + c) * 2 + 0] = u;
-            a.stats[((size_t)blockIdx.x * a.outC + (blockIdx.y * WM + m) * 16 + c) * 2 + 1] = v;
+            if (tid < WM * 16) {
+                const int m = tid >> 4, c = tid & 15;
+#pragma unroll
+                for (int g = 0; g < 4 / WM; ++g) { u += red[((g * WM + m) * 16 + c) * 2]; v += red[((g * WM + m) * 16 + c) * 2 + 1]; }
+            }
+            stat_rows_add(a.stats, a.outC, blockIdx.x, blockIdx.y * WM * 16, WM * 16, u, v);
         }
     }
 }
```

Result: no change. 785.0 million (-0.6%).
